# kwea123/nsff_pl

Hardware: AMD Instinct MI355X
Metric: ray-samples/sec (coarse+fine, static+dynamic) (higher is better)
Workload: dtype f16x3 (fp32 operands split into 2 halfs, 3 f16 MFMAs per product, fp32 accumulate; same 1e-4 parity as f32); 1 GPU; C2 (BASELINE.json configs[1]): static+dynamic NSFF, 1024 rays/GPU x (64 coarse + 64 importance -> 192 fine pts), train-mode fwd, fw/bw flow warp t+-1, perturb=1 noise_std=1, 8x256 MLPs, N_tau=48, all 47 outputs on device.  `value` is render_rays' throughput with autograd DISABLED (the train-mode FLAGS, inference launches: nothing kept for a backward pass); what a trainer's forward costs is aux.tra; rays_per_gpu=1024, N_samples=64, N_importance=64, parallelism=single GPU, field_launch=persistent (one workgroup per CU)

## Files before the change

### include/nsff_render.h

```cpp
#ifndef NSFF_RENDER_H
#define NSFF_RENDER_H

#include <stddef.h>
#include <stdint.h>

#ifdef __cplusplus
extern "C" {
#endif

#define NSFF_OK               0
#define NSFF_ERR_INVALID     -1
#define NSFF_ERR_NULL        -2
#define NSFF_ERR_ALIGN       -3
#define NSFF_ERR_HIP         -4

#define NSFF_ABI_VERSION      32
#define NSFF_RAW_STRIDE      16
#define NSFF_MAX_FREQS       24
#define NSFF_MAX_LAYERS       8


typedef struct NsffModelDesc {
    int32_t D;
    int32_t W;
    int32_t skip;
    int32_t in_xyz;
    int32_t in_dir;
    int32_t in_a;
    int32_t in_t;
    int32_t use_viewdir;
    int32_t has_transient;
    int32_t has_flow;
    float   flow_scale;
    int32_t skip_mask;
} NsffModelDesc;

static inline uint32_t nsff_skip_layers(const NsffModelDesc* d) {
    return d->skip_mask ? (uint32_t)d->skip_mask : (d->skip > 0 ? 1u << d->skip : 0u);
}

#define NSFF_PREC_F32        0
#define NSFF_PREC_F16X3      1

int nsff_packed_bytes(const NsffModelDesc* desc, int precision, size_t* bytes);

int nsff_param_count(const NsffModelDesc* desc);

int nsff_pack_weights(const NsffModelDesc* desc, int precision, const float* const* params,
                      void* packed, void* stream);

#define NSFF_PACK_SKIP_FOLD 1
int nsff_pack_weights_ex(const NsffModelDesc* desc, int precision, const float* const* params,
                         void* packed, int32_t flags, void* stream);
int nsff_fold_heads(const NsffModelDesc* desc, int precision, const float* const* params, void* packed, void* stream);

int nsff_posenc(const float* x, int64_t n_rows, const float* freqs_host, int n_freqs,
                float* out, void* stream);

int nsff_time_rows(const float* table, int64_t n_table, int32_t width, const int64_t* ts, int64_t n, int64_t max_t,
                   float* next, float* prev, void* stream);

int nsff_time_rows_backward(const float* g_cur, const float* g_next, const float* g_prev, const int64_t* ts, int64_t n,
                            int64_t max_t, int64_t n_table, int32_t width, float* d_table, void* stream);

typedef struct NsffFieldArgs {
    int64_t n_points;
    int32_t precision;
    int32_t tile_points;
    int32_t pts_per_ray;
    int32_t static_mode;
    int32_t transient_mode;
    int32_t flow_heads;
    const float* xyz;
    int32_t n_freqs;
    float   freqs[NSFF_MAX_FREQS];
    const float* dir_emb;
    const float* a_emb;
    const float* t_emb;
    const float* x_emb;
    int32_t ld_emb;
    int32_t off_xyz, off_dir, off_a, off_t;
    float*  raw;
    void*   save_acts;
    void*   save_xin;
    void*   save_masks;
    void*   save_side;
    const float* t_bias;
    int32_t t_bias_rows;
    int32_t reserved0;
    const float* s_bias;
    int32_t s_bias_rows;
    int32_t launch_form;
    int64_t save_lo_delta[3];
} NsffFieldArgs;

int nsff_field_query(const NsffModelDesc* desc, const void* packed,
                     const NsffFieldArgs* args, void* stream);

#define NSFF_MAX_TIME_BIAS_JOBS 4
typedef struct NsffTimeBiasJob {
    const NsffModelDesc* desc;
    const float* w[NSFF_MAX_LAYERS];
    const float* b[NSFF_MAX_LAYERS];
    const float* t_rows;
    float* out;
    const float* table;
    const int64_t* ts;
    int64_t n_table, max_t;
    int32_t delta, pad_;
    float* rows_out;
} NsffTimeBiasJob;
int nsff_time_bias_rows(const NsffModelDesc* desc);
int nsff_time_bias(const NsffTimeBiasJob* jobs, int32_t n_jobs, int64_t n_rays, void* stream);

#define NSFF_MAX_RNG_JOBS 12
typedef struct NsffRngJob {
    float*   out;
    int64_t  numel;
    uint64_t offset;
    int32_t  kind;
    uint32_t grid;
} NsffRngJob;
int nsff_rng_draws(const NsffRngJob* jobs, int32_t n_jobs, uint64_t seed, void* stream);
typedef struct NsffRngCoarse {
    const float* rays;
    const float* z_lin;
    float*       zs;
    float*       xyz;
    int32_t      n_samples;
    float        perturb;
    int32_t      job;
    int32_t      pad_;
} NsffRngCoarse;
int nsff_rng_draws_coarse(const NsffRngJob* jobs, int32_t n_jobs, uint64_t seed, const NsffRngCoarse* coarse, void* stream);

int nsff_side_bias(const NsffModelDesc* desc, const void* packed_f16x3, const float* w_dir, const float* dir_rows,
                   const float* a_rows, int64_t n_rays, float* out, void* stream);

int nsff_train_dims(const NsffModelDesc* desc, int32_t* xin_rows, int32_t* t_row0, int32_t* side_rows);
int nsff_bwd_packed_bytes(const NsffModelDesc* desc, size_t* bytes);
int nsff_pack_weights_bwd(const NsffModelDesc* desc, const float* const* params, void* packed, void* stream);
int nsff_pack_weights_bwd_ex(const NsffModelDesc* desc, const float* const* params, void* packed, const void* fwd_packed, void* stream);

typedef struct NsffFieldBwdArgs {
    int64_t n_points;
    int32_t static_mode;
    int32_t transient_mode;
    const float* d_raw;
    const float* raw;
    const float* gmax;
    const void*  masks;
    void*  dpre;
    void*  dhead;
    float* d_xin;
    float* d_side;
    int64_t dpre_lo_delta;
} NsffFieldBwdArgs;
int nsff_field_backward(const NsffModelDesc* desc, const void* packed_bwd, const NsffFieldBwdArgs* args, void* stream);
int nsff_last_bwd_kernel(void);
int nsff_last_bwd_grid(void);
int nsff_field_bwd_phase_program(const NsffModelDesc* desc, int32_t dynamic, int32_t want_xin, int64_t n_tiles, uint32_t* out,
                                 int32_t max_phases, uint32_t* seg_offsets, int32_t max_segs);

#define NSFF_BWD_LAUNCH_C    1
#define NSFF_BWD_LAUNCH_H3B  2
#define NSFF_BWD_LAUNCH_X3   3
int nsff_field_bwd_launch_plan(const NsffModelDesc* desc, const NsffFieldBwdArgs* args, int32_t n_cus, int32_t kernel_override,
                               int32_t persist, int32_t* out, int32_t max_launches);

int nsff_field_input_backward(const float* d_xin, int32_t xin_rows, int32_t t_row0, const float* xyz, int64_t n_rays,
                              int32_t pts_per_ray, const float* freqs_host, int32_t n_freqs, int32_t in_t, float* d_xyz,
                              float* d_t, void* stream);

typedef struct NsffWgradJob {
    const void* a;  const void* b;
    int32_t a_rows, b_rows;
    int64_t out_off;
    int32_t trunk, pad_;
    int64_t a_lo_delta, b_lo_delta;
} NsffWgradJob;
int64_t nsff_weight_grad_scratch(const NsffWgradJob* jobs, int32_t n_jobs, int64_t n_tiles, int32_t n_splits);
int nsff_weight_grad(const NsffWgradJob* jobs, int32_t n_jobs, int64_t n_tiles, int32_t n_splits,
                     float* scratch, float* out, float* bias, const float* gmax, void* stream);

typedef struct NsffGradMapEntry {
    int32_t dst;
    int32_t e_a, e_b;
    int16_t job_a, job_b;
} NsffGradMapEntry;
int nsff_weight_grad_accumulate(const NsffWgradJob* jobs, int32_t n_jobs, int64_t n_tiles, int32_t n_splits, float* scratch,
                                const NsffGradMapEntry* map, int64_t n_map, float* grad_base, const float* gmax, void* stream);

int nsff_weight_grad_accumulate_aux(const NsffWgradJob* jobs, int32_t n_jobs, int64_t n_tiles, int32_t n_splits, float* scratch,
                                    const NsffGradMapEntry* map, int64_t n_map, float* grad_base, float* aux, const float* gmax,
                                    void* stream);

typedef struct NsffFoldGradArgs {
    int32_t n_rows, pad_;
    const float* g; const float* gb;
    const float* w_final; const float* b_final;
    const float* w_head[16];
    float* d_w_head[16]; float* d_b_head[16];
    float* d_w_final; float* d_b_final;
} NsffFoldGradArgs;
int nsff_fold_grads(const NsffFoldGradArgs* args, void* stream);

typedef struct NsffFoldDenseArgs {
    int32_t n_rows, accumulate;
    int32_t ld_head, ld_dhead;
    const float* g; const float* g2; const float* gb; const float* gb2;
    const float* w_head; const float* w_final; const float* b_final;
    float* d_w_head; float* d_b_head; float* d_w_final; float* d_b_final;
} NsffFoldDenseArgs;
int nsff_fold_grads_dense(const NsffFoldDenseArgs* args, void* stream);

int nsff_absmax(const float* x, int64_t n, float* out, void* stream);
int nsff_absmax_raw(const float* d_raw, int64_t n_points, float* out16, void* stream);

int nsff_adam_step(float* param, const float* grad, float* exp_avg, float* exp_avg_sq, int64_t n, float* state,
                   const float* lr, double beta1, double beta2, double eps, double weight_decay, void* stream);

int nsff_adam_step_segments(float* param, const float* grad, float* exp_avg, float* exp_avg_sq, int64_t n, float* state,
                            const float* lr, double beta1, double beta2, double eps, double weight_decay,
                            const int64_t* seg_start, int n_seg, int32_t* seg_used, void* stream);

typedef struct NsffLossArgs {
    int64_t n_rays; int32_t n_samples; int32_t n_keep;
    int32_t n_frames; int32_t max_t;
    double  topk;
    int32_t thickness; int32_t pad_;
    const float* rgb_fine; const float* rgb_coarse;
    const float* depth_fine; const float* depth_coarse;
    const float* t_weights; const float* s_weights;
    const float* xyz_fw; const float* xyz_bw;
    const float* rgb_fw; const float* rgb_bw;
    const float* disocc_fw; const float* disocc_bw;
    const float* disoccs_fw; const float* disoccs_bw;
    const float* xyzs_fw_bw; const float* xyzs_bw_fw;
    const float* xyzs_fine; const float* xyzs_fw; const float* xyzs_bw;
    const float* rgbs; const float* disps;
    const int64_t* ts; const int64_t* cam_ids;
    const float* uv_fw; const float* uv_bw;
    const float* Ks; const float* Ps;
    const float* hyper;
    float* stats;
    float* terms;
    const float* term_w;
    const float* weights;
    float* per_ray;
    float* coef;
    float* g_rgb_fine; float* g_rgb_coarse; float* g_depth_fine; float* g_depth_coarse;
    float* g_t_weights; float* g_s_weights; float* g_xyz_fw; float* g_xyz_bw; float* g_rgb_fw; float* g_rgb_bw;
    float* g_xyzs_fw_bw; float* g_xyzs_bw_fw; float* g_xyzs_fw; float* g_xyzs_bw;
} NsffLossArgs;
int nsff_nerfw_loss(const NsffLossArgs* args, int mode, void* stream);
#define NSFF_LOSS_MAX_RAYS 1048576
size_t nsff_nerfw_loss_work_bytes(long long n_rays);
int nsff_nerfw_loss_ex(const NsffLossArgs* args, int mode, void* work, size_t work_bytes, void* stream);
int nsff_last_loss_path(void);

int nsff_coarse_samples(const float* rays, int64_t n_rays, const float* z_lin, int32_t n_samples,
                        float perturb, const float* perturb_rand,
                        float* zs, float* xyz, void* stream);

int nsff_fine_samples(const float* rays, int64_t n_rays, const float* z_lin, const float* zs_coarse,
                      int32_t n_samples, int32_t n_importance,
                      const float* weights_static, const float* weights_transient,
                      const float* u_static, const float* u_transient, int32_t u_per_ray,
                      float* samples_static, float* samples_transient,
                      float* zs_fine, float* xyz_fine, void* stream);

int nsff_sample_pdf(const float* bins, const float* weights, int64_t n_rays, int32_t n_bins_minus1,
                    const float* u, int32_t n_importance, int32_t u_per_ray, float eps,
                    float* samples, void* stream);

int nsff_warp_points(const float* raw, const float* xyz, const float* zs, int64_t n_points,
                     float z_far, float* xyz_fw, float* xyz_bw, void* stream);

int nsff_frame_rays(const float* K4_host, const float* c2w_host, int32_t H, int32_t W, float near, float shift_near,
                    int64_t first_pixel, int64_t n_pixels, float* rays, void* stream);

typedef struct NsffFrustumArgs {
    const float*   w2c;
    const int64_t* ts;
    float   K4[4];
    int32_t n_cams, n_frames, H, W;
} NsffFrustumArgs;

typedef struct NsffCompositeArgs {
    int64_t n_rays;
    int32_t n_samples;
    int32_t has_transient;
    int32_t has_rgb;
    int32_t flow_mode;
    int32_t want_disocc;
    float   noise_std;
    float   z_far;
    const float* raw;
    const float* raw_fw;
    const float* raw_bw;
    const float* zs;
    const float* xyz;
    const float* xyz_fw;
    const float* xyz_bw;
    const float* noise_static;
    const float* noise_transient;
    const float* noise_fw;
    const float* noise_bw;
    const float* visibility;
    float* static_rgbs;  float* transient_rgbs;
    float* flows_fw;     float* flows_bw;
    float* static_sigmas; float* transient_sigmas;
    float* static_alphas; float* transient_alphas;
    float* static_weights; float* transient_weights; float* weights;
    float* xyzs_fw_bw;   float* xyzs_bw_fw;
    float* disoccs_fw;   float* disoccs_bw;
    float* depth;  float* rgb;  float* transient_alpha;  float* transient_rgb;
    float* static_only_rgb;  float* static_only_depth;
    float* xyz_exp;  float* flow_fw_exp;  float* flow_bw_exp;  float* xyz_fw_exp;  float* xyz_bw_exp;
    float* rgb_fw;   float* rgb_bw;
    float* disocc_fw;  float* disocc_bw;
    NsffFrustumArgs vis;
} NsffCompositeArgs;

int nsff_composite(const NsffCompositeArgs* args, void* stream);

int nsff_frustum_visibility(const NsffFrustumArgs* vis, const float* xyz, int64_t n_points, float* vis_count,
                            void* stream);

typedef struct NsffSplatArgs {
    int32_t H, W, n_planes;
    float   K4[4];
    float   P[12];
    float   scale;
    const float* xyz;
    const float* flow;
    const float* rgb;
    const float* alpha;
    float*       accum;
    void*        work;
    int64_t      work_bytes;
} NsffSplatArgs;
int64_t nsff_splat_work_bytes(int32_t H, int32_t W, int32_t n_planes);
int nsff_splat_planes(const NsffSplatArgs* args, void* stream);

typedef struct NsffMpiArgs {
    int32_t H, W, n_planes;
    float   dt;
    const float* accum_fw;
    const float* accum_bw;
    const float* static_rgb;
    const float* static_alpha;
    const float* zs;
    float* rgb;
    float* depth;
} NsffMpiArgs;
int nsff_mpi_composite(const NsffMpiArgs* args, void* stream);

typedef struct NsffCompositeBwdArgs {
    int64_t n_rays;
    int32_t n_samples, has_transient, flow_mode;
    float   noise_std;
    const float* raw;  const float* raw_fw;  const float* raw_bw;
    const float* zs;   const float* xyz;     const float* f_fw;  const float* f_bw;
    const float* noise_static;  const float* noise_transient;  const float* noise_fw;  const float* noise_bw;
    const float* g_static_sigmas;  const float* g_transient_sigmas;
    const float* g_static_weights; const float* g_transient_weights;  const float* g_weights;
    const float* g_depth;  const float* g_rgb;  const float* g_transient_alpha;  const float* g_transient_rgb;
    const float* g_so_rgb; const float* g_so_depth;
    const float* g_xyz_exp;  const float* g_flow_fw_exp;  const float* g_flow_bw_exp;
    const float* g_rgb_fw;   const float* g_rgb_bw;
    float* scratch;
    float* d_raw;  float* d_raw_fw;  float* d_raw_bw;  float* d_f_fw;  float* d_f_bw;
} NsffCompositeBwdArgs;
int nsff_composite_backward(const NsffCompositeBwdArgs* args, void* stream);

typedef struct {
    int64_t n_points;
    const float* zs;
    float z_far;
    int32_t accumulate;
    int32_t col_a, col_b;
    int32_t pad_;
    const float* g_a[4];
    const float* g_b[4];
    float* out;
} NsffFlowGradArgs;
int nsff_flow_grad(const NsffFlowGradArgs* args, void* stream);

#define NSFF_RAY_RECORD      16

typedef struct NsffSsimArgs {
    int32_t n_frames, H, W, window;
    const float* gt;  const float* pred;  const uint8_t* mask;
    float* map;  float* mean_map;  double* sums;
    void* scratch;  int64_t scratch_bytes;
} NsffSsimArgs;
int64_t nsff_ssim_scratch_bytes(int32_t n_frames, int32_t H, int32_t W);
int nsff_ssim(const NsffSsimArgs* args, void* stream);

int nsff_cdf(const float* weights, int64_t n_frames, int64_t n, double* cdf, void* stream);

typedef struct NsffRayDrawArgs {
    int64_t n_frames, n_pixels, frame, batch;
    const float* records;  const double* cdf;  const float* u;
    float* rays;  float* rgbs;  int64_t* ts;  int64_t* cam_ids;  float* disps;  float* rays_mask;  float* uv_fw;  float* uv_bw;
    int64_t* rand_idx;
} NsffRayDrawArgs;
int nsff_ray_draw(const NsffRayDrawArgs* args, void* stream);

int nsff_prof_enable(int on);
int nsff_prof_collect(int64_t* launches, double* total_ms, double* total_flops, double* executed_flops);
int nsff_prof_collect_clock(int64_t* launches, double* total_ms, double* total_flops, double* executed_flops,
                            double* shader_ticks, double* ticks_ms);

#define NSFF_KERNEL_F32       1
#define NSFF_KERNEL_H3_64     2
#define NSFF_KERNEL_H3_8WAVE  3
#define NSFF_KERNEL_H3A       4
#define NSFF_KERNEL_H3_SAVE   5
#define NSFF_KERNEL_H3A_TBIAS 7
#define NSFF_KERNEL_H3A_SAVE  9
#define NSFF_KERNEL_H3A_SIDE  8
int         nsff_last_field_kernel(void);
int         nsff_last_field_grid(void);
int         nsff_field_phase_program(const NsffModelDesc* desc, int static_mode, int transient_mode, int fold_t, uint32_t* steps,
                             int* n_steps, int* n_static_steps, uint32_t* phases_static, uint32_t* phases_dynamic, int* n_phases);

#define NSFF_PLAN_WORDS 12
#define NSFF_LAUNCH_SIDE_TILE      1
#define NSFF_LAUNCH_H3_64          2
#define NSFF_LAUNCH_H3_64_SAVE     3
#define NSFF_LAUNCH_H3_8WAVE       4
#define NSFF_LAUNCH_H3_8WAVE_SAVE  5
#define NSFF_LAUNCH_H3A            6
#define NSFF_LAUNCH_H3A_SAVE       7
int         nsff_field_launch_plan(const NsffModelDesc* desc, const NsffFieldArgs* args, int32_t n_cus, int32_t no_persist,
                                   int32_t* out, int32_t max_launches);

#define NSFF_RANGE_ACT     0x1u
#define NSFF_RANGE_SAVED   0x2u
#define NSFF_RANGE_PARAMS  0x4u
#define NSFF_RANGE_CODES   0x8u
int         nsff_range_flags(uint32_t* out, int32_t clear, void* stream);

int         nsff_abi_version(void);
const char* nsff_last_hip_error(void);

#ifdef __cplusplus
}
#endif
#endif
```

### nsff_pl_amd/_lib.py

```python
import ctypes as C
import os

import torch

_HERE = os.path.dirname(os.path.abspath(__file__))
LIB_PATH = os.environ.get("NSFF_LIB") or os.path.join(_HERE, "libnsff_hip.so")

RAW_STRIDE = 16
ABI_VERSION = 32
MAX_FREQS = 24

_ERR = {-1: "NSFF_ERR_INVALID (bad shape/flag/unsupported architecture)",
        -2: "NSFF_ERR_NULL (required pointer missing)",
        -3: "NSFF_ERR_ALIGN (pointer not 16-byte aligned)",
        -4: "NSFF_ERR_HIP"}

_fp = C.c_void_p


class ModelDesc(C.Structure):
    _fields_ = [("D", C.c_int32), ("W", C.c_int32), ("skip", C.c_int32),
                ("in_xyz", C.c_int32), ("in_dir", C.c_int32), ("in_a", C.c_int32),
                ("in_t", C.c_int32), ("use_viewdir", C.c_int32),
                ("has_transient", C.c_int32), ("has_flow", C.c_int32),
                ("flow_scale", C.c_float), ("skip_mask", C.c_int32)]


class FieldArgs(C.Structure):
    _fields_ = [("n_points", C.c_int64), ("precision", C.c_int32), ("tile_points", C.c_int32),
                ("pts_per_ray", C.c_int32),
                ("static_mode", C.c_int32), ("transient_mode", C.c_int32),
                ("flow_heads", C.c_int32),
                ("xyz", _fp), ("n_freqs", C.c_int32), ("freqs", C.c_float * MAX_FREQS),
                ("dir_emb", _fp), ("a_emb", _fp), ("t_emb", _fp),
                ("x_emb", _fp), ("ld_emb", C.c_int32),
                ("off_xyz", C.c_int32), ("off_dir", C.c_int32), ("off_a", C.c_int32),
                ("off_t", C.c_int32), ("raw", _fp), ("save_acts", _fp), ("save_xin", _fp), ("save_masks", _fp),
                ("save_side", _fp), ("t_bias", _fp), ("t_bias_rows", C.c_int32), ("reserved0", C.c_int32),
                ("s_bias", _fp), ("s_bias_rows", C.c_int32), ("launch_form", C.c_int32), ("save_lo_delta", C.c_int64 * 3)]


class TimeBiasJob(C.Structure):
    _fields_ = [("desc", C.POINTER(ModelDesc)), ("w", _fp * 8), ("b", _fp * 8), ("t_rows", _fp), ("out", _fp),
                ("table", _fp), ("ts", _fp), ("n_table", C.c_int64), ("max_t", C.c_int64), ("delta", C.c_int32), ("pad_", C.c_int32),
                ("rows_out", _fp)]


MAX_TIME_BIAS_JOBS = 4


class RngJob(C.Structure):
    _fields_ = [("out", _fp), ("numel", C.c_int64), ("offset", C.c_uint64), ("kind", C.c_int32), ("grid", C.c_uint32)]


MAX_RNG_JOBS = 12


class RngCoarse(C.Structure):
    _fields_ = [("rays", _fp), ("z_lin", _fp), ("zs", _fp), ("xyz", _fp), ("n_samples", C.c_int32), ("perturb", C.c_float),
                ("job", C.c_int32), ("pad_", C.c_int32)]


_COMPOSITE_PTRS_IN = ["raw", "raw_fw", "raw_bw", "zs", "xyz", "xyz_fw", "xyz_bw",
                      "noise_static", "noise_transient", "noise_fw", "noise_bw", "visibility"]
_COMPOSITE_PTRS_OUT = ["static_rgbs", "transient_rgbs", "flows_fw", "flows_bw",
                       "static_sigmas", "transient_sigmas", "static_alphas", "transient_alphas",
                       "static_weights", "transient_weights", "weights",
                       "xyzs_fw_bw", "xyzs_bw_fw", "disoccs_fw", "disoccs_bw",
                       "depth", "rgb", "transient_alpha", "transient_rgb",
                       "static_only_rgb", "static_only_depth",
                       "xyz_exp", "flow_fw_exp", "flow_bw_exp", "xyz_fw_exp", "xyz_bw_exp",
                       "rgb_fw", "rgb_bw", "disocc_fw", "disocc_bw"]


class FrustumArgs(C.Structure):
    _fields_ = [("w2c", _fp), ("ts", _fp), ("K4", C.c_float * 4), ("n_cams", C.c_int32), ("n_frames", C.c_int32),
                ("H", C.c_int32), ("W", C.c_int32)]


class CompositeArgs(C.Structure):
    _fields_ = ([("n_rays", C.c_int64), ("n_samples", C.c_int32), ("has_transient", C.c_int32),
                 ("has_rgb", C.c_int32), ("flow_mode", C.c_int32), ("want_disocc", C.c_int32),
                 ("noise_std", C.c_float), ("z_far", C.c_float)]
                + [(n, _fp) for n in _COMPOSITE_PTRS_IN]
                + [(n, _fp) for n in _COMPOSITE_PTRS_OUT]
                + [("vis", FrustumArgs)])


_CBWD_IN = ["raw", "raw_fw", "raw_bw", "zs", "xyz", "f_fw", "f_bw", "noise_static", "noise_transient", "noise_fw", "noise_bw"]
_CBWD_G = ["g_static_sigmas", "g_transient_sigmas", "g_static_weights", "g_transient_weights", "g_weights", "g_depth",
           "g_rgb", "g_transient_alpha", "g_transient_rgb", "g_so_rgb", "g_so_depth", "g_xyz_exp", "g_flow_fw_exp",
           "g_flow_bw_exp", "g_rgb_fw", "g_rgb_bw"]
_CBWD_OUT = ["scratch", "d_raw", "d_raw_fw", "d_raw_bw", "d_f_fw", "d_f_bw"]


class CompositeBwdArgs(C.Structure):
    _fields_ = ([("n_rays", C.c_int64), ("n_samples", C.c_int32), ("has_transient", C.c_int32), ("flow_mode", C.c_int32),
                 ("noise_std", C.c_float)] + [(n, _fp) for n in _CBWD_IN + _CBWD_G + _CBWD_OUT])


class FieldBwdArgs(C.Structure):
    _fields_ = [("n_points", C.c_int64), ("static_mode", C.c_int32), ("transient_mode", C.c_int32),
                ("d_raw", _fp), ("raw", _fp), ("gmax", _fp), ("masks", _fp), ("dpre", _fp), ("dhead", _fp),
                ("d_xin", _fp), ("d_side", _fp), ("dpre_lo_delta", C.c_int64)]


class WgradJob(C.Structure):
    _fields_ = [("a", _fp), ("b", _fp), ("a_rows", C.c_int32), ("b_rows", C.c_int32), ("out_off", C.c_int64), ("trunk", C.c_int32),
                ("pad_", C.c_int32), ("a_lo_delta", C.c_int64), ("b_lo_delta", C.c_int64)]


class FoldGradArgs(C.Structure):
    _fields_ = [("n_rows", C.c_int32), ("pad_", C.c_int32), ("g", _fp), ("gb", _fp), ("w_final", _fp), ("b_final", _fp),
                ("w_head", _fp * 16), ("d_w_head", _fp * 16), ("d_b_head", _fp * 16), ("d_w_final", _fp), ("d_b_final", _fp)]


class FoldDenseArgs(C.Structure):
    _fields_ = [("n_rows", C.c_int32), ("accumulate", C.c_int32), ("ld_head", C.c_int32), ("ld_dhead", C.c_int32),
                ("g", _fp), ("g2", _fp), ("gb", _fp), ("gb2", _fp), ("w_head", _fp), ("w_final", _fp), ("b_final", _fp),
                ("d_w_head", _fp), ("d_b_head", _fp), ("d_w_final", _fp), ("d_b_final", _fp)]


class SplatArgs(C.Structure):
    _fields_ = [("H", C.c_int32), ("W", C.c_int32), ("n_planes", C.c_int32), ("K4", C.c_float * 4),
                ("P", C.c_float * 12), ("scale", C.c_float),
                ("xyz", _fp), ("flow", _fp), ("rgb", _fp), ("alpha", _fp), ("accum", _fp), ("work", _fp),
                ("work_bytes", C.c_int64)]


class MpiArgs(C.Structure):
    _fields_ = [("H", C.c_int32), ("W", C.c_int32), ("n_planes", C.c_int32), ("dt", C.c_float),
                ("accum_fw", _fp), ("accum_bw", _fp), ("static_rgb", _fp), ("static_alpha", _fp), ("zs", _fp),
                ("rgb", _fp), ("depth", _fp)]


_LOSS_IN = ["rgb_fine", "rgb_coarse", "depth_fine", "depth_coarse", "t_weights", "s_weights", "xyz_fw", "xyz_bw", "rgb_fw",
            "rgb_bw", "disocc_fw", "disocc_bw", "disoccs_fw", "disoccs_bw", "xyzs_fw_bw", "xyzs_bw_fw", "xyzs_fine",
            "xyzs_fw", "xyzs_bw", "rgbs", "disps", "ts", "cam_ids", "uv_fw", "uv_bw", "Ks", "Ps", "hyper", "stats", "terms",
            "term_w"]
LOSS_GRADS = ["g_rgb_fine", "g_rgb_coarse", "g_depth_fine", "g_depth_coarse", "g_t_weights", "g_s_weights", "g_xyz_fw",
              "g_xyz_bw", "g_rgb_fw", "g_rgb_bw", "g_xyzs_fw_bw", "g_xyzs_bw_fw", "g_xyzs_fw", "g_xyzs_bw"]


class LossArgs(C.Structure):
    _fields_ = ([("n_rays", C.c_int64), ("n_samples", C.c_int32), ("n_keep", C.c_int32), ("n_frames", C.c_int32),
                 ("max_t", C.c_int32), ("topk", C.c_double), ("thickness", C.c_int32), ("pad_", C.c_int32)]
                + [(n, _fp) for n in _LOSS_IN] + [("weights", _fp), ("per_ray", _fp), ("coef", _fp)]
                + [(n, _fp) for n in LOSS_GRADS])


class FlowGradArgs(C.Structure):
    _fields_ = [("n_points", C.c_int64), ("zs", _fp), ("z_far", C.c_float), ("accumulate", C.c_int32), ("col_a", C.c_int32),
                ("col_b", C.c_int32), ("pad_", C.c_int32), ("g_a", _fp * 4), ("g_b", _fp * 4), ("out", _fp)]


class SsimArgs(C.Structure):
    _fields_ = [("n_frames", C.c_int32), ("H", C.c_int32), ("W", C.c_int32), ("window", C.c_int32),
                ("gt", _fp), ("pred", _fp), ("mask", _fp), ("map", _fp), ("mean_map", _fp), ("sums", _fp),
                ("scratch", _fp), ("scratch_bytes", C.c_int64)]


RAY_RECORD = 16
_DRAW_OUT = ["rays", "rgbs", "ts", "cam_ids", "disps", "rays_mask", "uv_fw", "uv_bw", "rand_idx"]


class RayDrawArgs(C.Structure):
    _fields_ = ([("n_frames", C.c_int64), ("n_pixels", C.c_int64), ("frame", C.c_int64), ("batch", C.c_int64),
                 ("records", _fp), ("cdf", _fp), ("u", _fp)] + [(n, _fp) for n in _DRAW_OUT])


_SIGNATURES = {
    "nsff_abi_version": (C.c_int, []),
    "nsff_range_flags": (C.c_int, [_fp, C.c_int32, _fp]),
    "nsff_last_field_kernel": (C.c_int, []),
    "nsff_last_field_grid": (C.c_int, []),
    "nsff_field_phase_program": (C.c_int, [C.POINTER(ModelDesc), C.c_int, C.c_int, C.c_int, C.POINTER(C.c_uint32), C.POINTER(C.c_int),
                                   C.POINTER(C.c_int), C.POINTER(C.c_uint32), C.POINTER(C.c_uint32), C.POINTER(C.c_int)]),
    "nsff_field_launch_plan": (C.c_int, [C.POINTER(ModelDesc), C.POINTER(FieldArgs), C.c_int32, C.c_int32, C.POINTER(C.c_int32), C.c_int32]),
    "nsff_time_bias_rows": (C.c_int, [C.POINTER(ModelDesc)]),
    "nsff_time_bias": (C.c_int, [C.POINTER(TimeBiasJob), C.c_int32, C.c_int64, C.c_void_p]),
    "nsff_rng_draws": (C.c_int, [C.POINTER(RngJob), C.c_int32, C.c_uint64, C.c_void_p]),
    "nsff_rng_draws_coarse": (C.c_int, [C.POINTER(RngJob), C.c_int32, C.c_uint64, C.POINTER(RngCoarse), C.c_void_p]),
    "nsff_side_bias": (C.c_int, [C.POINTER(ModelDesc), _fp, _fp, _fp, _fp, C.c_int64, _fp, C.c_void_p]),
    "nsff_last_hip_error": (C.c_char_p, []),
    "nsff_packed_bytes": (C.c_int, [C.POINTER(ModelDesc), C.c_int, C.POINTER(C.c_size_t)]),
    "nsff_param_count": (C.c_int, [C.POINTER(ModelDesc)]),
    "nsff_pack_weights": (C.c_int, [C.POINTER(ModelDesc), C.c_int, C.POINTER(_fp), _fp, _fp]),
    "nsff_pack_weights_ex": (C.c_int, [C.POINTER(ModelDesc), C.c_int, C.POINTER(_fp), _fp, C.c_int32, _fp]),
    "nsff_fold_heads": (C.c_int, [C.POINTER(ModelDesc), C.c_int, C.POINTER(_fp), _fp, _fp]),
    "nsff_posenc": (C.c_int, [_fp, C.c_int64, C.POINTER(C.c_float), C.c_int, _fp, _fp]),
    "nsff_time_rows": (C.c_int, [_fp, C.c_int64, C.c_int32, _fp, C.c_int64, C.c_int64, _fp, _fp, _fp]),
    "nsff_time_rows_backward": (C.c_int, [_fp, _fp, _fp, _fp, C.c_int64, C.c_int64, C.c_int64, C.c_int32, _fp, _fp]),
    "nsff_field_query": (C.c_int, [C.POINTER(ModelDesc), _fp, C.POINTER(FieldArgs), _fp]),
    "nsff_coarse_samples": (C.c_int, [_fp, C.c_int64, _fp, C.c_int32, C.c_float, _fp, _fp, _fp, _fp]),
    "nsff_fine_samples": (C.c_int, [_fp, C.c_int64, _fp, _fp, C.c_int32, C.c_int32, _fp, _fp, _fp, _fp,
                                    C.c_int32, _fp, _fp, _fp, _fp, _fp]),
    "nsff_sample_pdf": (C.c_int, [_fp, _fp, C.c_int64, C.c_int32, _fp, C.c_int32, C.c_int32,
                                  C.c_float, _fp, _fp]),
    "nsff_warp_points": (C.c_int, [_fp, _fp, _fp, C.c_int64, C.c_float, _fp, _fp, _fp]),
    "nsff_composite": (C.c_int, [C.POINTER(CompositeArgs), _fp]),
    "nsff_frustum_visibility": (C.c_int, [C.POINTER(FrustumArgs), _fp, C.c_int64, _fp, _fp]),
    "nsff_frame_rays": (C.c_int, [C.POINTER(C.c_float), C.POINTER(C.c_float), C.c_int32, C.c_int32, C.c_float,
                                  C.c_float, C.c_int64, C.c_int64, _fp, _fp]),
    "nsff_bwd_packed_bytes": (C.c_int, [C.POINTER(ModelDesc), C.POINTER(C.c_size_t)]),
    "nsff_pack_weights_bwd": (C.c_int, [C.POINTER(ModelDesc), C.POINTER(_fp), _fp, _fp]),
    "nsff_field_backward": (C.c_int, [C.POINTER(ModelDesc), _fp, C.POINTER(FieldBwdArgs), _fp]),
    "nsff_field_input_backward": (C.c_int, [_fp, C.c_int32, C.c_int32, _fp, C.c_int64, C.c_int32, C.POINTER(C.c_float), C.c_int32,
                                            C.c_int32, _fp, _fp, _fp]),
    "nsff_train_dims": (C.c_int, [C.POINTER(ModelDesc), C.POINTER(C.c_int32), C.POINTER(C.c_int32), C.POINTER(C.c_int32)]),
    "nsff_weight_grad_scratch": (C.c_int64, [C.POINTER(WgradJob), C.c_int32, C.c_int64, C.c_int32]),
    "nsff_weight_grad": (C.c_int, [C.POINTER(WgradJob), C.c_int32, C.c_int64, C.c_int32, _fp, _fp, _fp, _fp, _fp]),
    "nsff_weight_grad_accumulate": (C.c_int, [C.POINTER(WgradJob), C.c_int32, C.c_int64, C.c_int32, _fp, _fp, C.c_int64,
                                              _fp, _fp, _fp]),
    "nsff_weight_grad_accumulate_aux": (C.c_int, [C.POINTER(WgradJob), C.c_int32, C.c_int64, C.c_int32, _fp, _fp, C.c_int64,
                                                  _fp, _fp, _fp, _fp]),
    "nsff_absmax_raw": (C.c_int, [_fp, C.c_int64, _fp, _fp]),
    "nsff_last_bwd_kernel": (C.c_int, []),
    "nsff_last_bwd_grid": (C.c_int, []),
    "nsff_field_bwd_phase_program": (C.c_int, [C.POINTER(ModelDesc), C.c_int32, C.c_int32, C.c_int64, C.POINTER(C.c_uint32), C.c_int32,
                                                C.POINTER(C.c_uint32), C.c_int32]),
    "nsff_field_bwd_launch_plan": (C.c_int, [C.POINTER(ModelDesc), C.POINTER(FieldBwdArgs), C.c_int32, C.c_int32, C.c_int32,
                                             C.POINTER(C.c_int32), C.c_int32]),
    "nsff_fold_grads": (C.c_int, [C.POINTER(FoldGradArgs), _fp]),
    "nsff_fold_grads_dense": (C.c_int, [C.POINTER(FoldDenseArgs), _fp]),
    "nsff_pack_weights_bwd_ex": (C.c_int, [C.POINTER(ModelDesc), C.POINTER(_fp), _fp, _fp, _fp]),
    "nsff_absmax": (C.c_int, [_fp, C.c_int64, _fp, _fp]),
    "nsff_adam_step": (C.c_int, [_fp, _fp, _fp, _fp, C.c_int64, _fp, _fp, C.c_double, C.c_double, C.c_double, C.c_double, _fp]),
    "nsff_adam_step_segments": (C.c_int, [_fp, _fp, _fp, _fp, C.c_int64, _fp, _fp, C.c_double, C.c_double, C.c_double, C.c_double,
                                          _fp, C.c_int, _fp, _fp]),
    "nsff_composite_backward": (C.c_int, [C.POINTER(CompositeBwdArgs), _fp]),
    "nsff_flow_grad": (C.c_int, [C.POINTER(FlowGradArgs), _fp]),
    "nsff_nerfw_loss": (C.c_int, [C.POINTER(LossArgs), C.c_int, _fp]),
    "nsff_nerfw_loss_work_bytes": (C.c_size_t, [C.c_longlong]),
    "nsff_nerfw_loss_ex": (C.c_int, [C.POINTER(LossArgs), C.c_int, _fp, C.c_size_t, _fp]),
    "nsff_last_loss_path": (C.c_int, []),
    "nsff_splat_planes": (C.c_int, [C.POINTER(SplatArgs), _fp]),
    "nsff_splat_work_bytes": (C.c_int64, [C.c_int32, C.c_int32, C.c_int32]),
    "nsff_mpi_composite": (C.c_int, [C.POINTER(MpiArgs), _fp]),
    "nsff_ssim_scratch_bytes": (C.c_int64, [C.c_int32, C.c_int32, C.c_int32]),
    "nsff_ssim": (C.c_int, [C.POINTER(SsimArgs), _fp]),
    "nsff_cdf": (C.c_int, [_fp, C.c_int64, C.c_int64, _fp, _fp]),
    "nsff_ray_draw": (C.c_int, [C.POINTER(RayDrawArgs), _fp]),
    "nsff_prof_enable": (C.c_int, [C.c_int]),
    "nsff_prof_collect": (C.c_int, [C.POINTER(C.c_int64), C.POINTER(C.c_double), C.POINTER(C.c_double), C.POINTER(C.c_double)]),
    "nsff_prof_collect_clock": (C.c_int, [C.POINTER(C.c_int64)] + [C.POINTER(C.c_double)] * 5),
}
EXPORTED_SYMBOLS = tuple(_SIGNATURES)

_lib = None


def load():
    global _lib
    if _lib is None:
        if not os.path.exists(LIB_PATH):
            raise RuntimeError(
                f"{LIB_PATH} is missing: build it with `python -c 'import __graft_entry__ as g; g.build()'` "
                "(or `make -C nsff_pl_amd/csrc`).  There is no CPU fallback for the render path.")
        lib = C.CDLL(LIB_PATH)
        for name, (res, args) in _SIGNATURES.items():
            fn = getattr(lib, name)
            fn.restype, fn.argtypes = res, args
        if lib.nsff_abi_version() != ABI_VERSION:
            raise RuntimeError("libnsff_hip.so ABI version mismatch")
        _lib = lib
    return _lib


def _check(rc, what):
    if rc != 0:
        msg = _ERR.get(rc, f"error {rc}")
        if rc == -4:
            msg += ": " + load().nsff_last_hip_error().decode()
        raise RuntimeError(f"{what} failed: {msg}")


def require_gpu_tensor(t, what):
    if not isinstance(t, torch.Tensor) or not t.is_cuda:
        raise RuntimeError(f"{what} must be a GPU tensor: the NSFF render path runs only on the "
                           "HIP kernels of libnsff_hip.so (no CPU fallback)")


def _ptr(t):
    if t is None:
        return None
    assert t.is_cuda and t.dtype == torch.float32 and t.is_contiguous(), "need contiguous fp32 GPU tensor"
    return t.data_ptr()


def _stream():
    return torch.cuda.current_stream().cuda_stream


def model_desc(model):
    if model.W != 256:
        raise RuntimeError(f"unsupported NeRF architecture: W={model.W} (the gfx950 field kernels tile W=256 trunks "
                           "into 4 x 64-neuron wave blocks; other widths are not built)")
    skips = sorted(set(int(s) for s in model.skips))
    if not 2 <= model.D <= 8 or any(not 1 <= s < model.D for s in skips):
        raise RuntimeError(f"unsupported NeRF architecture: D={model.D}, skips={list(model.skips)} (need 2 <= D <= 8 "
                           "and every skip layer in 1..D-1; a skip at layer 0 would concatenate the input with itself)")
    mask = sum(1 << s for s in skips)
    return ModelDesc(D=model.D, W=model.W, skip=skips[0] if len(skips) == 1 else 0, skip_mask=mask if len(skips) != 1 else 0,
                     in_xyz=model.in_channels_xyz,
                     in_dir=model.in_channels_dir,
                     in_a=model.in_channels_a if model.use_viewdir else 0,
                     in_t=model.in_channels_t, use_viewdir=int(model.use_viewdir),
                     has_transient=int(model.encode_transient),
                     has_flow=int(getattr(model, "has_flow_heads", hasattr(model, "transient_flow_fw"))),
                     flow_scale=float(getattr(model, "flow_scale", 0.0)))


def param_list(model):
    def lin(m):
        layer = m[0] if isinstance(m, torch.nn.Sequential) else m
        return [layer.weight, layer.bias]
    out = []
    for i in range(model.D):
        out += lin(getattr(model, f"static_xyz_encoding_{i + 1}"))
    out += lin(model.static_xyz_encoding_final)
    if model.use_viewdir:
        out += lin(model.static_dir_encoding)
    out += lin(model.static_sigma) + lin(model.static_rgb)
    if model.encode_transient:
        for i in range(model.D):
            out += lin(getattr(model, f"transient_xyz_encoding_{i + 1}"))
        out += lin(model.transient_xyz_encoding_final)
        out += lin(model.transient_sigma) + lin(model.transient_rgb)
        if hasattr(model, "transient_flow_fw"):
            out += lin(model.transient_flow_fw) + lin(model.transient_flow_bw)
    return out


def packed_bytes(desc, precision=0):
    n = C.c_size_t(0)
    _check(load().nsff_packed_bytes(C.byref(desc), int(precision), C.byref(n)), "nsff_packed_bytes")
    return n.value


PACK_SKIP_FOLD = 1


def pack_weights(desc, params, packed, precision=0, fold=True):
    lib = load()
    if lib.nsff_param_count(C.byref(desc)) != len(params):
        raise RuntimeError("parameter list does not match the model description")
    keep = [p.detach().contiguous().float() for p in params]
    for p in keep:
        require_gpu_tensor(p, "model parameter")
    arr = (_fp * len(keep))(*[p.data_ptr() for p in keep])
    _check(lib.nsff_pack_weights_ex(C.byref(desc), int(precision), arr, _ptr(packed), 0 if fold else PACK_SKIP_FOLD,
                                    _stream()), "nsff_pack_weights_ex")
    return keep


def fold_heads(desc, params, packed, precision):
    keep = [p.detach().contiguous().float() for p in params]
    arr = (_fp * len(keep))(*[p.data_ptr() for p in keep])
    _check(load().nsff_fold_heads(C.byref(desc), int(precision), arr, _ptr(packed), _stream()), "nsff_fold_heads")
    return keep


def time_rows_backward(g_cur, g_next, g_prev, ts, max_t, n_table):
    gs = [None if g is None else g.contiguous() for g in (g_cur, g_next, g_prev)]
    width = next(g for g in gs if g is not None).shape[1]
    assert ts.dtype == torch.int64 and ts.is_cuda and ts.is_contiguous()
    d = torch.empty(int(n_table), width, device=ts.device)
    _check(load().nsff_time_rows_backward(_ptr(gs[0]), _ptr(gs[1]), _ptr(gs[2]), C.c_void_p(ts.data_ptr()), ts.shape[0],
                                          int(max_t), int(n_table), width, _ptr(d), _stream()), "nsff_time_rows_backward")
    return d


def time_rows(table, ts, max_t, want_next=True, want_prev=True):
    n, width = ts.shape[0], table.shape[1]
    if want_next and want_prev:
        both = torch.empty(2, n, width, device=table.device)
        nxt, prv = both[0], both[1]
    else:
        nxt = torch.empty(n, width, device=table.device) if want_next else None
        prv = torch.empty(n, width, device=table.device) if want_prev else None
    assert ts.dtype == torch.int64 and ts.is_cuda and ts.is_contiguous()
    _check(load().nsff_time_rows(_ptr(table), table.shape[0], width, C.c_void_p(ts.data_ptr()), n, int(max_t),
                                 _ptr(nxt), _ptr(prv), _stream()), "nsff_time_rows")
    return nxt, prv


def posenc(x, freqs, out):
    f = [float(v) for v in freqs]
    arr = (C.c_float * len(f))(*f)
    _check(load().nsff_posenc(_ptr(x), x.shape[0], arr, len(f), _ptr(out), _stream()), "nsff_posenc")


def field_query(model, raw, n_points, pts_per_ray, static_mode, transient_mode, flow_heads=0,
                xyz=None, freqs=None, dir_emb=None, a_emb=None, t_emb=None,
                x_emb=None, emb_offsets=(0, -1, -1, -1), save_acts=None, save_xin=None, save_masks=None, save_side=None,
                precision=None, t_bias=None, s_bias=None, save_lo=False):
    from . import config
    desc = model_desc(model)
    prec = config.precision_code(model) if precision is None else precision
    saves = not (save_acts is None and save_xin is None and save_masks is None and save_side is None)
    packed = model.packed(prec)
    a = FieldArgs()
    a.precision, a.tile_points = prec, config.get_tile_points()
    a.launch_form = 0 if config.get_persistent() else 1
    a.n_points, a.pts_per_ray = int(n_points), int(pts_per_ray)
    a.static_mode, a.transient_mode, a.flow_heads = int(static_mode), int(transient_mode), int(flow_heads)
    a.xyz = _ptr(xyz)
    if freqs is not None:
        f = [float(v) for v in freqs]
        if len(f) > MAX_FREQS:
            raise RuntimeError("too many embedding frequencies")
        a.n_freqs = len(f)
        for i, v in enumerate(f):
            a.freqs[i] = v
    a.dir_emb, a.a_emb, a.t_emb = _ptr(dir_emb), _ptr(a_emb), _ptr(t_emb)
    a.x_emb = _ptr(x_emb)
    a.ld_emb = int(x_emb.shape[1]) if x_emb is not None else 0
    a.off_xyz, a.off_dir, a.off_a, a.off_t = [int(v) for v in emb_offsets]
    a.raw = _ptr(raw)
    a.save_acts = None if save_acts is None else save_acts.data_ptr()
    a.save_xin = None if save_xin is None else save_xin.data_ptr()
    a.save_masks = None if save_masks is None else save_masks.data_ptr()
    a.save_side = None if save_side is None else save_side.data_ptr()
    if save_lo:
        for i, t in enumerate((save_acts, save_xin, save_side)):
            a.save_lo_delta[i] = 0 if t is None else lo_delta(t)
    if t_bias is not None:
        a.t_bias, a.t_bias_rows = _ptr(t_bias), int(t_bias.shape[1])
    if s_bias is not None:
        a.s_bias, a.s_bias_rows = _ptr(s_bias), int(s_bias.shape[1])
    _check(load().nsff_field_query(C.byref(desc), _ptr(packed), C.byref(a), _stream()), "nsff_field_query")


def lo_delta(t):
    n = t.numel()
    if t.untyped_storage().nbytes() < (t.storage_offset() + 2 * n) * t.element_size():
        raise RuntimeError("three-product backward: this buffer has no remainder plane behind it (field_grad.alloc_saves(..., x3=True))")
    return n


def side_bias(model, dir_rows, a_rows=None):
    from . import config
    desc = model_desc(model)
    n_rays = int(dir_rows.shape[0])
    assert dir_rows.shape == (n_rays, desc.in_dir) and (desc.in_a == 0 or (a_rows is not None and a_rows.shape == (n_rays, desc.in_a)))
    packed = model.packed(config.PRECISIONS["f16x3"])
    w = model.static_dir_encoding[0].weight.detach()
    out = torch.empty(n_rays, 1, 256, device=dir_rows.device, dtype=torch.float32)
    _check(load().nsff_side_bias(C.byref(desc), _ptr(packed), _ptr(w), _ptr(dir_rows), _ptr(a_rows) if desc.in_a > 0 else None,
                                 n_rays, _ptr(out), _stream()), "nsff_side_bias")
    return out


_DEVICE_RNG_GEOMETRY = {}


def fused_draws(plan, device, values=True, coarse=None):
    dev = torch.device(device)
    idx = dev.index if dev.index is not None else torch.cuda.current_device()
    if idx not in _DEVICE_RNG_GEOMETRY:
        p = torch.cuda.get_device_properties(idx)
        _DEVICE_RNG_GEOMETRY[idx] = p.multi_processor_count * (p.max_threads_per_multi_processor // 256)
    max_grid = _DEVICE_RNG_GEOMETRY[idx]
    gen = torch.cuda.default_generators[idx]
    seed, offset = gen.initial_seed(), gen.get_offset()
    wanted = values if isinstance(values, (list, tuple)) else [bool(values)] * len(plan)
    sizes = []
    for kind, shape in plan:
        n = 1
        for s in shape:
            n *= int(s)
        sizes.append(n)
    total = sum(n for n, w in zip(sizes, wanted) if w)
    buf = torch.empty(max(total, 1), device=dev, dtype=torch.float32)
    outs, jobs, at = [], [], 0
    for (kind, shape), numel, want in zip(plan, sizes, wanted):
        if numel == 0:
            outs.append(torch.empty(*shape, device=dev, dtype=torch.float32))
            continue
        grid = min(max_grid, (numel + 255) // 256)
        if coarse is not None and not outs and not want:
            jobs.append((None, numel, offset, 0, grid))
            outs.append(None)
        elif want:
            t = buf[at:at + numel].view(*shape)
            at += numel
            jobs.append((t, numel, offset, 1 if kind == "randn" else 0, grid))
            outs.append(t)
        else:
            outs.append(None)
        offset += ((numel - 1) // (1024 * grid) + 1) * 4
    hook = None
    if coarse is not None:
        rays, z_lin, perturb, zs, xyz = coarse
        assert plan and plan[0][0] == "rand" and tuple(plan[0][1]) == (rays.shape[0], z_lin.shape[0]) and perturb > 0
        if sizes[0]:
            hook = RngCoarse(_ptr(rays), _ptr(z_lin), _ptr(zs), _ptr(xyz), int(z_lin.shape[0]), float(perturb), 0, 0)
    for k in range(0, len(jobs), MAX_RNG_JOBS):
        part = jobs[k:k + MAX_RNG_JOBS]
        arr = (RngJob * len(part))()
        for j, (t, numel, off, kind, grid) in enumerate(part):
            arr[j].out, arr[j].numel, arr[j].offset, arr[j].kind, arr[j].grid = (None if t is None else t.data_ptr()), numel, off, kind, grid
        with torch.cuda.device(idx):
            _check(load().nsff_rng_draws_coarse(arr, len(part), seed, C.byref(hook) if (hook is not None and k == 0) else None, _stream()),
                   "nsff_rng_draws")
    gen.set_offset(offset)
    return outs


_FUSED_DRAWS_OK = {}


def fused_draws_match_torch(device):
    dev = torch.device(device)
    idx = dev.index if dev.index is not None else torch.cuda.current_device()
    if idx in _FUSED_DRAWS_OK:
        return _FUSED_DRAWS_OK[idx]
    if torch.cuda.is_current_stream_capturing():
        return False
    gen = torch.cuda.default_generators[idx]
    state = gen.get_state()
    ok = True
    try:
        plan = [("rand", (7, 64)), ("randn", (1031,)), ("rand", (3, 5, 2)), ("randn", (70000,)), ("rand", (300001,))]
        gen.manual_seed(0x5EED1234)
        gen.set_offset(8)
        mine = fused_draws(plan, torch.device("cuda", idx))
        end_mine = gen.get_offset()
        gen.manual_seed(0x5EED1234)
        gen.set_offset(8)
        with torch.cuda.device(idx):
            ref = [(torch.rand if k == "rand" else torch.randn)(*shape, device=torch.device("cuda", idx)) for k, shape in plan]
        end_ref = gen.get_offset()
        ok = end_mine == end_ref and all(torch.equal(a.view(torch.int32), b.view(torch.int32)) for a, b in zip(mine, ref))
    except Exception:
        ok = False
    finally:
        gen.set_state(state)
    if not ok:
        import warnings
        warnings.warn("nsff_pl_amd: the fused generator kernel (nsff_rng_draws) no longer reproduces torch.rand / torch.randn on "
                      f"cuda:{idx} (torch {torch.__version__}); render_rays draws with the torch calls instead (slower by ~1 %, same "
                      "numbers as the reference)")
    _FUSED_DRAWS_OK[idx] = ok
    return ok


def time_bias_rows(model):
    return load().nsff_time_bias_rows(C.byref(model_desc(model)))


def time_bias(jobs, index=None):
    assert 1 <= len(jobs) <= MAX_TIME_BIAS_JOBS
    arr = (TimeBiasJob * len(jobs))()
    keep, outs, per_model, pair = [], [], {}, None
    rows_of = {}
    if index is not None:
        table, ts, max_t = index
        assert ts.dtype == torch.int64 and ts.is_cuda and ts.is_contiguous() and ts.dim() == 1, "ts: one int64 frame index per ray"
        n_rays, width = int(ts.shape[0]), int(table.shape[1])
        deltas = sorted({int(d) for _, d in jobs})
        if 1 in deltas and -1 in deltas:
            both = torch.empty(2, n_rays, width, device=table.device, dtype=torch.float32)
            rows_of[1], rows_of[-1] = both[0], both[1]
        for d in deltas:
            if d not in rows_of:
                rows_of[d] = torch.empty(n_rays, width, device=table.device, dtype=torch.float32)
        written = set()
    else:
        n_rays = int(jobs[0][1].shape[0])
    for j, (model, t_rows) in enumerate(jobs):
        if id(model) not in per_model:
            desc = model_desc(model)
            lins = [getattr(model, f"transient_xyz_encoding_{l + 1}")[0] for l in [0] + sorted(set(int(v) for v in model.skips))]
            wb = [(m.weight.detach(), m.bias.detach()) for m in lins]
            for w, b in wb:
                _ptr(w), _ptr(b)
            per_model[id(model)] = (desc, C.pointer(desc), wb)
        desc, pdesc, wb = per_model[id(model)]
        if index is not None:
            delta, t_rows = int(t_rows), None
            assert width == desc.in_t
        else:
            assert t_rows.shape == (n_rays, desc.in_t)
        dev = wb[0][0].device
        if j + 1 < len(jobs) and jobs[j + 1][0] is model and pair is None:
            pair = torch.empty(2, n_rays, len(wb), 256, device=dev, dtype=torch.float32)
            out = pair[0]
        elif pair is not None:
            out, pair = pair[1], None
        else:
            out = torch.empty(n_rays, len(wb), 256, device=dev, dtype=torch.float32)
        arr[j].desc = pdesc
        for i, (w, b) in enumerate(wb):
            arr[j].w[i], arr[j].b[i] = w.data_ptr(), b.data_ptr()
        arr[j].t_rows, arr[j].out = _ptr(t_rows), _ptr(out)
        if index is not None:
            arr[j].table, arr[j].ts = _ptr(table), ts.data_ptr()
            arr[j].n_table, arr[j].max_t, arr[j].delta = int(table.shape[0]), int(max_t), delta
            if delta not in written:
                arr[j].rows_out = _ptr(rows_of[delta])
                written.add(delta)
        outs.append(out)
    keep.append(per_model)
    _check(load().nsff_time_bias(arr, len(jobs), n_rays, _stream()), "nsff_time_bias")
    return outs if index is None else (outs, rows_of)


def coarse_samples(rays, z_lin, perturb, perturb_rand, zs, xyz):
    _check(load().nsff_coarse_samples(_ptr(rays), rays.shape[0], _ptr(z_lin), z_lin.shape[0],
                                      float(perturb), _ptr(perturb_rand), _ptr(zs), _ptr(xyz), _stream()),
           "nsff_coarse_samples")


def fine_samples(rays, z_lin, zs_coarse, n_importance, w_static, w_transient, u_static, u_transient,
                 u_per_ray, samples_static, samples_transient, zs_fine, xyz_fine):
    _check(load().nsff_fine_samples(_ptr(rays), rays.shape[0], _ptr(z_lin), _ptr(zs_coarse),
                                    z_lin.shape[0], int(n_importance), _ptr(w_static), _ptr(w_transient),
                                    _ptr(u_static), _ptr(u_transient), int(u_per_ray),
                                    _ptr(samples_static), _ptr(samples_transient),
                                    _ptr(zs_fine), _ptr(xyz_fine), _stream()), "nsff_fine_samples")


def sample_pdf(bins, weights, u, u_per_ray, eps, samples):
    _check(load().nsff_sample_pdf(_ptr(bins), _ptr(weights), weights.shape[0], weights.shape[1],
                                  _ptr(u), samples.shape[1], int(u_per_ray), float(eps),
                                  _ptr(samples), _stream()), "nsff_sample_pdf")


def warp_points(raw, xyz, zs, z_far, xyz_fw, xyz_bw):
    _check(load().nsff_warp_points(_ptr(raw), _ptr(xyz), _ptr(zs), zs.numel(), float(z_far),
                                   _ptr(xyz_fw), _ptr(xyz_bw), _stream()), "nsff_warp_points")


def frustum_args(w2c, ts, K4, n_cams, n_frames, H, W):
    assert w2c.is_cuda and w2c.dtype == torch.float32 and w2c.is_contiguous() and w2c.shape == (n_cams * n_frames, 12)
    assert ts.is_cuda and ts.dtype == torch.int64 and ts.is_contiguous() and ts.numel() >= 1
    a = FrustumArgs(w2c=w2c.data_ptr(), ts=ts.data_ptr(), n_cams=int(n_cams), n_frames=int(n_frames), H=int(H), W=int(W))
    a.K4[:] = [float(v) for v in K4]
    a._keep = (w2c, ts)
    return a


def frustum_visibility(vis, xyz, out):
    _check(load().nsff_frustum_visibility(C.byref(vis), _ptr(xyz), xyz.shape[0], _ptr(out), _stream()),
           "nsff_frustum_visibility")


def composite(vis=None, **kw):
    a = CompositeArgs()
    for k, v in kw.items():
        if k in _COMPOSITE_PTRS_IN or k in _COMPOSITE_PTRS_OUT:
            setattr(a, k, _ptr(v))
        else:
            setattr(a, k, v)
    if vis is not None:
        a.vis = vis
    _check(load().nsff_composite(C.byref(a), _stream()), "nsff_composite")


def frame_rays(K4, c2w12, H, W, near, shift_near, first, count, rays):
    k = (C.c_float * 4)(*[float(v) for v in K4])
    m = (C.c_float * 12)(*[float(v) for v in c2w12])
    _check(load().nsff_frame_rays(k, m, int(H), int(W), float(near), float(shift_near), int(first), int(count),
                                  _ptr(rays), _stream()), "nsff_frame_rays")


BWD_PACK = 100


def bwd_packed_bytes(desc):
    n = C.c_size_t(0)
    _check(load().nsff_bwd_packed_bytes(C.byref(desc), C.byref(n)), "nsff_bwd_packed_bytes")
    return n.value


def pack_weights_bwd(desc, params, packed, fwd_packed=None):
    arr = (_fp * len(params))(*[p.data_ptr() for p in params])
    _check(load().nsff_pack_weights_bwd_ex(C.byref(desc), arr, _ptr(packed), _ptr(fwd_packed), _stream()), "nsff_pack_weights_bwd_ex")


def last_bwd_kernel():
    return {0: "c", 1: "h3b", 2: "c+h3b", 3: "x3"}[load().nsff_last_bwd_kernel()]


def last_bwd_grid():
    return load().nsff_last_bwd_grid()


PLAN_WORDS = 12


def field_launch_plan(desc, args, n_cus, no_persist=False):
    out = (C.c_int32 * (3 * PLAN_WORDS))()
    code = load().nsff_field_launch_plan(C.byref(desc), C.byref(args), int(n_cus), int(bool(no_persist)), out, 3)
    recs = [list(out[i * PLAN_WORDS:(i + 1) * PLAN_WORDS]) for i in range(3)]
    return code, [r for r in recs if r[0] != 0]


def field_bwd_launch_plan(desc, args, n_cus, kernel_override=None, persist=True):
    out = (C.c_int32 * (2 * PLAN_WORDS))()
    code = load().nsff_field_bwd_launch_plan(C.byref(desc), C.byref(args), int(n_cus), ord(kernel_override) if kernel_override else 0,
                                                      int(bool(persist)), out, 2)
    recs = [list(out[i * PLAN_WORDS:(i + 1) * PLAN_WORDS]) for i in range(2)]
    return code, [r for r in recs if r[0] != 0]


def field_bwd_phase_program(model, dynamic, want_xin, n_tiles, max_phases=32):
    import numpy as np
    desc = model_desc(model)
    out = (C.c_uint32 * (8 * max_phases))()
    segs = (C.c_uint32 * 48)()
    n = load().nsff_field_bwd_phase_program(C.byref(desc), 1 if dynamic else 0, 1 if want_xin else 0, int(n_tiles), out, max_phases, segs, 48)
    if n < 0:
        raise RuntimeError(f"nsff_field_bwd_phase_program failed ({n})")
    offs = np.array(list(segs), np.uint32)
    return (np.array(list(out), np.uint32).reshape(max_phases, 8)[:n] if n > 0 else None), offs


def field_backward(model, n_points, static, transient, d_raw, raw, gmax, masks, dpre, dhead, d_xin, d_side=None, x3=False):
    desc = model_desc(model)
    a = FieldBwdArgs(n_points=int(n_points), static_mode=2 if static else 0, transient_mode=2 if transient else 0,
                     d_raw=_ptr(d_raw), raw=_ptr(raw), gmax=_ptr(gmax), masks=masks.data_ptr(), dpre=dpre.data_ptr(),
                     dhead=dhead.data_ptr(), d_xin=_ptr(d_xin), d_side=_ptr(d_side), dpre_lo_delta=lo_delta(dpre) if x3 else 0)
    _check(load().nsff_field_backward(C.byref(desc), _ptr(model.packed(BWD_PACK)), C.byref(a), _stream()),
           "nsff_field_backward")


def train_dims(model):
    desc = model_desc(model)
    xr, t0, sr = C.c_int32(0), C.c_int32(0), C.c_int32(0)
    _check(load().nsff_train_dims(C.byref(desc), C.byref(xr), C.byref(t0), C.byref(sr)), "nsff_train_dims")
    return xr.value, t0.value, sr.value


def field_input_backward(d_xin, t_row0, xyz, pts_per_ray, freqs, in_t, want_xyz, want_t):
    P, xin_rows = d_xin.shape
    n_rays = P // pts_per_ray
    d_xyz = torch.empty(P, 3, device=d_xin.device) if want_xyz else None
    d_t = torch.empty(n_rays, in_t, device=d_xin.device) if want_t else None
    f = [float(v) for v in freqs]
    arr = (C.c_float * max(len(f), 1))(*f)
    _check(load().nsff_field_input_backward(_ptr(d_xin), int(xin_rows), int(t_row0), _ptr(xyz), n_rays, int(pts_per_ray), arr,
                                            len(f), int(in_t), _ptr(d_xyz), _ptr(d_t), _stream()), "nsff_field_input_backward")
    return d_xyz, d_t


def _wgrad_jobs(jobs, with_off):
    return (WgradJob * len(jobs))(*[WgradJob(a=j[0], b=j[1], a_rows=j[2], b_rows=j[3], out_off=j[4] if with_off else 0, trunk=j[5],
                                             a_lo_delta=j[6] if len(j) > 6 else 0, b_lo_delta=j[7] if len(j) > 7 else 0) for j in jobs])


def weight_grad(jobs, n_tiles, n_splits, out, bias, gmax):
    arr = _wgrad_jobs(jobs, True)
    n = load().nsff_weight_grad_scratch(arr, len(jobs), int(n_tiles), int(n_splits))
    if n < 0:
        raise RuntimeError("nsff_weight_grad_scratch failed")
    scratch = torch.empty(n, device=out.device)
    _check(load().nsff_weight_grad(arr, len(jobs), int(n_tiles), int(n_splits), _ptr(scratch), _ptr(out), _ptr(bias),
                                   _ptr(gmax), _stream()), "nsff_weight_grad")


def weight_grad_accumulate(jobs, n_tiles, n_splits, grad_map, grad_base_ptr, gmax, aux=None):
    arr = _wgrad_jobs(jobs, False)
    n = load().nsff_weight_grad_scratch(arr, len(jobs), int(n_tiles), int(n_splits))
    if n < 0:
        raise RuntimeError("nsff_weight_grad_scratch failed")
    assert grad_map.dtype == torch.int32 and grad_map.is_contiguous() and grad_map.shape[1] == 4
    scratch = torch.empty(n, device=gmax.device)
    _check(load().nsff_weight_grad_accumulate_aux(arr, len(jobs), int(n_tiles), int(n_splits), _ptr(scratch),
                                                  C.c_void_p(grad_map.data_ptr()), grad_map.shape[0], C.c_void_p(grad_base_ptr),
                                                  _ptr(aux), _ptr(gmax), _stream()), "nsff_weight_grad_accumulate_aux")
    return scratch


def fold_grads(g, gb, w_final, b_final, head_rows, d_w_final, d_b_final):
    a = FoldGradArgs(n_rows=len(head_rows), g=_ptr(g), gb=_ptr(gb), w_final=_ptr(w_final), b_final=_ptr(b_final),
                     d_w_final=_ptr(d_w_final), d_b_final=_ptr(d_b_final))
    for r, (w, dw, db) in enumerate(head_rows):
        a.w_head[r], a.d_w_head[r], a.d_b_head[r] = w.data_ptr(), dw.data_ptr(), db.data_ptr()
    _check(load().nsff_fold_grads(C.byref(a), _stream()), "nsff_fold_grads")


def fold_grads_dense(g, gb, w_head, w_final, b_final, d_w_head, d_b_head, d_w_final, d_b_final, accumulate, g2=None, gb2=None):
    R = int(g.shape[0])
    for t in (g, g2, gb, gb2, w_final, b_final, d_w_final, d_b_final, d_b_head):
        assert t is None or (t.is_cuda and t.dtype == torch.float32 and t.is_contiguous())
    for t in (w_head, d_w_head):
        assert t.is_cuda and t.dtype == torch.float32 and t.shape[0] == R and t.shape[1] == 256 and t.stride(1) == 1
    a = FoldDenseArgs(n_rows=R, accumulate=1 if accumulate else 0, ld_head=int(w_head.stride(0)), ld_dhead=int(d_w_head.stride(0)),
                      g=g.data_ptr(), g2=None if g2 is None else g2.data_ptr(), gb=gb.data_ptr(), gb2=None if gb2 is None else gb2.data_ptr(),
                      w_head=w_head.data_ptr(), w_final=w_final.data_ptr(), b_final=b_final.data_ptr(), d_w_head=d_w_head.data_ptr(),
                      d_b_head=d_b_head.data_ptr(), d_w_final=d_w_final.data_ptr(), d_b_final=d_b_final.data_ptr())
    _check(load().nsff_fold_grads_dense(C.byref(a), _stream()), "nsff_fold_grads_dense")


def absmax(x):
    x = x.contiguous()
    if x.dim() == 2 and x.shape[1] == RAW_STRIDE:
        out = torch.empty(RAW_STRIDE, device=x.device, dtype=torch.float32)
        _check(load().nsff_absmax_raw(_ptr(x), x.shape[0], _ptr(out), _stream()), "nsff_absmax_raw")
        return out
    out = torch.empty((), device=x.device, dtype=torch.float32)
    _check(load().nsff_absmax(_ptr(x), x.numel(), _ptr(out), _stream()), "nsff_absmax")
    return out


def adam_step(param, grad, exp_avg, exp_avg_sq, state, lr, beta1, beta2, eps, weight_decay, seg_start=None, seg_used=None):
    if seg_start is None:
        _check(load().nsff_adam_step(_ptr(param), _ptr(grad), _ptr(exp_avg), _ptr(exp_avg_sq), param.numel(), _ptr(state), _ptr(lr),
                                     float(beta1), float(beta2), float(eps), float(weight_decay), _stream()), "nsff_adam_step")
        return
    _check(load().nsff_adam_step_segments(_ptr(param), _ptr(grad), _ptr(exp_avg), _ptr(exp_avg_sq), param.numel(), _ptr(state),
                                          _ptr(lr), float(beta1), float(beta2), float(eps), float(weight_decay),
                                          C.c_void_p(seg_start.data_ptr()), int(seg_used.numel()),
                                          C.c_void_p(seg_used.data_ptr()), _stream()),
           "nsff_adam_step_segments")


def composite_backward(n_rays, n_samples, has_transient, flow_mode, noise_std, **tensors):
    a = CompositeBwdArgs(n_rays=int(n_rays), n_samples=int(n_samples), has_transient=int(has_transient),
                         flow_mode=int(flow_mode), noise_std=float(noise_std))
    for k, v in tensors.items():
        setattr(a, k, _ptr(v))
    _check(load().nsff_composite_backward(C.byref(a), _stream()), "nsff_composite_backward")


def flow_grad(zs, z_far, out, accumulate, col_a=-1, g_a=(), col_b=-1, g_b=()):
    a = FlowGradArgs(n_points=int(out.shape[0]), zs=_ptr(zs), z_far=float(z_far), accumulate=int(bool(accumulate)),
                     col_a=int(col_a), col_b=int(col_b), out=_ptr(out))
    if len(g_a) > 4 or len(g_b) > 4:
        raise ValueError("flow_grad: at most four cotangents per group")
    keep = [g.contiguous() for g in list(g_a) + list(g_b)]
    for i, g in enumerate(keep[:len(g_a)]):
        a.g_a[i] = _ptr(g)
    for i, g in enumerate(keep[len(g_a):]):
        a.g_b[i] = _ptr(g)
    _check(load().nsff_flow_grad(C.byref(a), _stream()), "nsff_flow_grad")


def nerfw_loss(mode, n_rays, n_samples, n_keep, n_frames, max_t, topk=1.0, thickness=1, work=None, **tensors):
    a = LossArgs(n_rays=int(n_rays), n_samples=int(n_samples), n_keep=int(n_keep), n_frames=int(n_frames), max_t=int(max_t),
                 topk=float(topk), thickness=int(thickness))
    for k, v in tensors.items():
        if v is None:
            continue
        if not torch.is_tensor(v):
            raise TypeError(f"nerfw_loss: {k} must be a tensor")
        if v.dtype == torch.int64:
            assert v.is_cuda and v.is_contiguous()
            setattr(a, k, v.data_ptr())
        else:
            setattr(a, k, _ptr(v))
    if work is None:
        _check(load().nsff_nerfw_loss(C.byref(a), int(mode), _stream()), "nsff_nerfw_loss")
        return
    if not (torch.is_tensor(work) and work.is_cuda and work.dtype == torch.uint8 and work.is_contiguous()):
        raise TypeError("nerfw_loss: work must be a contiguous uint8 GPU tensor")
    _check(load().nsff_nerfw_loss_ex(C.byref(a), int(mode), work.data_ptr(), work.numel(), _stream()), "nsff_nerfw_loss_ex")


LOSS_MAX_RAYS = 1 << 20


def nerfw_loss_work_bytes(n_rays):
    return int(load().nsff_nerfw_loss_work_bytes(int(n_rays)))


def last_loss_path():
    return int(load().nsff_last_loss_path())


def splat_work_bytes(H, W, S):
    return int(load().nsff_splat_work_bytes(int(H), int(W), int(S)))


def splat_planes(H, W, S, K4, P12, scale, xyz, flow, rgb, alpha, accum, work=None):
    a = SplatArgs(H=int(H), W=int(W), n_planes=int(S), scale=float(scale), xyz=_ptr(xyz), flow=_ptr(flow),
                  rgb=_ptr(rgb), alpha=_ptr(alpha), accum=_ptr(accum))
    if work is not None:
        assert work.is_cuda and work.is_contiguous() and work.dtype == torch.uint8
        a.work, a.work_bytes = work.data_ptr(), work.numel()
    a.K4[:] = [float(v) for v in K4]
    a.P[:] = [float(v) for v in P12]
    _check(load().nsff_splat_planes(C.byref(a), _stream()), "nsff_splat_planes")


def mpi_composite(H, W, S, dt, accum_fw, accum_bw, static_rgb, static_alpha, zs, rgb, depth):
    a = MpiArgs(H=int(H), W=int(W), n_planes=int(S), dt=float(dt), accum_fw=_ptr(accum_fw), accum_bw=_ptr(accum_bw),
                static_rgb=_ptr(static_rgb), static_alpha=_ptr(static_alpha), zs=_ptr(zs), rgb=_ptr(rgb),
                depth=_ptr(depth))
    _check(load().nsff_mpi_composite(C.byref(a), _stream()), "nsff_mpi_composite")


KERNEL_NAMES = {0: None, 1: "f32", 2: "h3_64", 3: "h3_8wave", 4: "h3a", 5: "h3_save", 7: "h3a_tb", 8: "h3a_side", 9: "h3a_save"}


def _dptr(t, dtype, what):
    if t is None:
        return None
    require_gpu_tensor(t, what)
    if t.dtype != dtype or not t.is_contiguous():
        raise RuntimeError(f"{what}: need a contiguous {dtype} tensor, got {t.dtype}"
                           f"{'' if t.is_contiguous() else ' (non-contiguous)'}")
    return t.data_ptr()


def ssim_scratch_bytes(n_frames, H, W):
    return int(load().nsff_ssim_scratch_bytes(int(n_frames), int(H), int(W)))


def ssim(gt, pred, mask=None, map=None, mean_map=None, sums=None, scratch=None):
    require_gpu_tensor(gt, "ssim: image_gt")
    require_gpu_tensor(pred, "ssim: image_pred")
    if gt.dim() != 4 or gt.shape[-1] != 3 or pred.shape != gt.shape:
        raise RuntimeError(f"ssim: need (F, H, W, 3) image pairs of one shape, got {tuple(gt.shape)} and {tuple(pred.shape)}")
    F, H, W = (int(v) for v in gt.shape[:3])
    if mask is not None and mask.dtype == torch.bool:
        mask = mask.view(torch.uint8)
    if sums is not None and scratch is None:
        scratch = torch.zeros(max(ssim_scratch_bytes(F, H, W), 16), dtype=torch.uint8, device=gt.device)
    a = SsimArgs(n_frames=F, H=H, W=W, window=11, gt=_dptr(gt, torch.float32, "ssim: image_gt"),
                 pred=_dptr(pred, torch.float32, "ssim: image_pred"), mask=_dptr(mask, torch.uint8, "ssim: mask"),
                 map=_dptr(map, torch.float32, "ssim: map"), mean_map=_dptr(mean_map, torch.float32, "ssim: mean_map"),
                 sums=_dptr(sums, torch.float64, "ssim: sums"), scratch=_dptr(scratch, torch.uint8, "ssim: scratch"),
                 scratch_bytes=0 if scratch is None else scratch.numel())
    for t, n in ((mask, F * H * W), (map, F * H * W * 3), (mean_map, F * H * W), (sums, F * 3)):
        if t is not None and t.numel() != n:
            raise RuntimeError(f"ssim: an output / mask has {t.numel()} elements, expected {n}")
    with torch.cuda.device(gt.device):
        _check(load().nsff_ssim(C.byref(a), _stream()), "nsff_ssim")


def cdf(weights, out):
    F, N = weights.shape
    if tuple(out.shape) != (F, N):
        raise RuntimeError("cdf: output shape mismatch")
    with torch.cuda.device(weights.device):
        _check(load().nsff_cdf(_dptr(weights, torch.float32, "cdf: weights"), F, N, _dptr(out, torch.float64, "cdf: out"),
                               _stream()), "nsff_cdf")


def ray_draw(records, frame, u, cdf, out):
    NF, NP = int(records.shape[0]), int(records.shape[1])
    if records.dim() != 3 or records.shape[2] != RAY_RECORD:
        raise RuntimeError(f"ray_draw: records must be (N_frames, N_pixels, {RAY_RECORD})")
    B = int(u.numel())
    a = RayDrawArgs(n_frames=NF, n_pixels=NP, frame=int(frame), batch=B, records=_dptr(records, torch.float32, "ray_draw: records"),
                    cdf=_dptr(cdf, torch.float64, "ray_draw: cdf"), u=_dptr(u, torch.float32, "ray_draw: u"))
    for n in _DRAW_OUT:
        t = out.get(n)
        setattr(a, n, _dptr(t, torch.int64 if n in ("ts", "cam_ids", "rand_idx") else torch.float32, f"ray_draw: {n}"))
    with torch.cuda.device(records.device):
        _check(load().nsff_ray_draw(C.byref(a), _stream()), "nsff_ray_draw")


def range_flags(out, clear):
    assert out.is_cuda and out.dtype == torch.int32 and out.numel() >= 1
    _check(load().nsff_range_flags(out.data_ptr(), 1 if clear else 0, _stream()), "nsff_range_flags")


def last_field_kernel():
    return KERNEL_NAMES[load().nsff_last_field_kernel()]


def last_field_grid():
    return int(load().nsff_last_field_grid())


def h3a_program(model, static_mode, transient_mode, fold_t=False, side_fold=False, persist=False):
    desc = model_desc(model)
    steps = (C.c_uint32 * (28 * 4))()
    ps, pd = (C.c_uint32 * (36 * 8))(), (C.c_uint32 * (36 * 8))()
    n, ns, nph = C.c_int(0), C.c_int(0), (C.c_int * 2)()
    _check(load().nsff_field_phase_program(C.byref(desc), int(static_mode), int(transient_mode), int(bool(fold_t)) | (2 if side_fold else 0) | (4 if persist else 0), steps, C.byref(n), C.byref(ns), ps, pd, nph),
           "nsff_field_phase_program")
    out = []
    for i in range(n.value):
        w, b, packed = steps[4 * i], steps[4 * i + 1], steps[4 * i + 2]
        out.append((w, None if b == 0xFFFFFFFF else b, packed & 0xFF, (packed >> 8) & 0xFF, (packed >> 16) & 0xFF, packed >> 24))
    rows = lambda arr, k: [[int(arr[8 * i + j]) for j in range(8)] for i in range(k)]
    return out, ns.value, rows(ps, nph[0]), rows(pd, nph[1])


def prof_enable(on):
    _check(load().nsff_prof_enable(int(bool(on))), "nsff_prof_enable")


def prof_collect():
    n, ms, fl, ex, tk, tms = C.c_int64(0), C.c_double(0), C.c_double(0), C.c_double(0), C.c_double(0), C.c_double(0)
    _check(load().nsff_prof_collect_clock(C.byref(n), C.byref(ms), C.byref(fl), C.byref(ex), C.byref(tk), C.byref(tms)),
           "nsff_prof_collect_clock")
    ghz = tk.value / tms.value * 1e-6 if tms.value > 0 else None
    if ghz is not None and not (0.5 < ghz < 3.0):
        ghz = None
    return n.value, ms.value, fl.value, ex.value, ghz
```

### nsff_pl_amd/csrc/rays.hip

```cpp
#include <hip/hip_runtime.h>
#include <cstdlib>
#include "nsff_common.h"

namespace {

constexpr int WAVES_PER_BLOCK = 4;
constexpr int RS = NSFF_RAW_STRIDE;

__device__ __forceinline__ float wave_sum(float v) {
#pragma unroll
    for (int off = 32; off > 0; off >>= 1) v += __shfl_xor(v, off);
    return v;
}

__device__ __forceinline__ float wave_scan_mul(float v, int lane) {
#pragma unroll
    for (int off = 1; off < 64; off <<= 1) {
        const float u = __shfl_up(v, off);
        if (lane >= off) v *= u;
    }
    return v;
}
__device__ __forceinline__ float wave_scan_add(float v, int lane) {
#pragma unroll
    for (int off = 1; off < 64; off <<= 1) {
        const float u = __shfl_up(v, off);
        if (lane >= off) v += u;
    }
    return v;
}

__device__ __forceinline__ float softplus(float x) { return x > 20.f ? x : log1pf(expf(x)); }

__global__ void coarse_samples_kernel(const float* __restrict__ rays, long long n_rays,
                                      const float* __restrict__ z_lin, int S, float perturb,
                                      const float* __restrict__ rnd, float* __restrict__ zs,
                                      float* __restrict__ xyz) {
    const long long idx = (long long)blockIdx.x * blockDim.x + threadIdx.x;
    if (idx >= n_rays * S) return;
    const long long n = idx / S;
    const int i = (int)(idx - n * S);
    float z = z_lin[i];
    if (perturb > 0.f) {
        const float lower = i > 0 ? 0.5f * (z_lin[i - 1] + z_lin[i]) : z_lin[0];
        const float upper = i < S - 1 ? 0.5f * (z_lin[i] + z_lin[i + 1]) : z_lin[S - 1];
        z = lower + (upper - lower) * (perturb * rnd[idx]);
    }
    zs[idx] = z;
    const float* r = rays + n * 6;
#pragma unroll
    for (int c = 0; c < 3; ++c) xyz[idx * 3 + c] = r[c] + r[3 + c] * z;
}

__device__ __forceinline__ void sample_pdf_ray(const float* w, const float* bins, int M, float eps,
                                               const float* u, int n_imp, float* cdf,
                                               float* out_a, float* out_b, int lane, bool active) {
    float part = 0.f;
    for (int j = lane; j < M; j += 64) part += (active ? w[j] : 0.f) + eps;
    const float total = wave_sum(part);
    float carry = 0.f;
    if (lane == 0) cdf[0] = 0.f;
    for (int base = 0; base < M; base += 64) {
        const int j = base + lane;
        const float pdf = j < M ? ((active ? w[j] : 0.f) + eps) / total : 0.f;
        const float inc = wave_scan_add(pdf, lane) + carry;
        if (j < M) cdf[j + 1] = inc;
        carry = __shfl(inc, 63);
    }
    __syncthreads();
    for (int k = lane; k < n_imp; k += 64) {
        const float uk = active ? u[k] : 0.f;
        int lo = 0, hi = M + 1;
        while (lo < hi) {
            const int mid = (lo + hi) >> 1;
            if (cdf[mid] <= uk) lo = mid + 1; else hi = mid;
        }
        const int below = max(lo - 1, 0), above = min(lo, M);
        const float cb = cdf[below], ca = cdf[above];
        const float bb = bins[below], ba = bins[above];
        float denom = ca - cb;
        if (denom < eps) denom = 1.f;
        const float s = bb + (uk - cb) / denom * (ba - bb);
        if (active) {
            if (out_a) out_a[k] = s;
            if (out_b) out_b[k] = s;
        }
    }
    __syncthreads();
}

struct FineArgs {
    const float* rays; long long n_rays; const float* z_lin; const float* zs_coarse;
    int S, n_imp;
    const float* w_static; const float* w_transient;
    const float* u_static; const float* u_transient; int u_per_ray;
    float* samples_static; float* samples_transient;
    float* zs_fine; float* xyz_fine;
};

__global__ __launch_bounds__(64 * WAVES_PER_BLOCK) void fine_samples_kernel(const FineArgs a) {
    extern __shared__ __attribute__((aligned(16))) float smem[];
    const int lane = threadIdx.x & 63, wave = threadIdx.x >> 6, tid = threadIdx.x;
    constexpr int T = 64 * WAVES_PER_BLOCK;
    const long long ray = blockIdx.x;
    const int S = a.S, n_imp = a.n_imp;
    const int k_sets = a.w_transient ? 2 : 1;
    const int Sf = S + k_sets * n_imp;
    float* cdf = smem + wave * S;
    float* bins = smem + WAVES_PER_BLOCK * S;
    float* merged = bins + ((S + 3) & ~3);
    for (int j = tid; j < S - 1; j += T) bins[j] = 0.5f * (a.z_lin[j] + a.z_lin[j + 1]);
    for (int j = tid; j < S; j += T) merged[j] = a.zs_coarse[ray * S + j];
    __syncthreads();
    {
        const bool mine = wave < k_sets;
        const int set = mine ? wave : 0;
        const float* w = (set == 0 ? a.w_static : a.w_transient) + ray * S + 1;
        const float* ub = set == 0 ? a.u_static : a.u_transient;
        const float* u = a.u_per_ray ? ub + ray * n_imp : ub;
        float* keep = set == 0 ? a.samples_static : a.samples_transient;
        sample_pdf_ray(w, bins, S - 2, 1e-5f, u, n_imp, cdf, merged + S + set * n_imp,
                       keep ? keep + ray * n_imp : nullptr, lane, mine);
    }
    const float* r = a.rays + ray * 6;
    const float o0 = r[0], o1 = r[1], o2 = r[2], d0 = r[3], d1 = r[4], d2 = r[5];
    for (int i = tid; i < Sf; i += T) {
        const float v = merged[i];
        int rank = 0;
        int j = 0;
        for (; j + 4 <= Sf; j += 4) {
            const float4 o = *reinterpret_cast<const float4*>(merged + j);
            rank += (o.x < v || (o.x == v && j < i)) ? 1 : 0;
            rank += (o.y < v || (o.y == v && j + 1 < i)) ? 1 : 0;
            rank += (o.z < v || (o.z == v && j + 2 < i)) ? 1 : 0;
            rank += (o.w < v || (o.w == v && j + 3 < i)) ? 1 : 0;
        }
        for (; j < Sf; ++j) {
            const float o = merged[j];
            rank += (o < v || (o == v && j < i)) ? 1 : 0;
        }
        const long long dst = ray * Sf + rank;
        a.zs_fine[dst] = v;
        a.xyz_fine[dst * 3 + 0] = o0 + d0 * v;
        a.xyz_fine[dst * 3 + 1] = o1 + d1 * v;
        a.xyz_fine[dst * 3 + 2] = o2 + d2 * v;
    }
}

struct PdfArgs {
    const float* bins; const float* weights; long long n_rays; int M;
    const float* u; int n_imp; int u_per_ray; float eps; float* samples;
};

__global__ __launch_bounds__(64 * WAVES_PER_BLOCK) void sample_pdf_kernel(const PdfArgs a) {
    extern __shared__ __attribute__((aligned(16))) float smem[];
    const int lane = threadIdx.x & 63, wave = threadIdx.x >> 6;
    const long long ray_raw = (long long)blockIdx.x * WAVES_PER_BLOCK + wave;
    const bool active = ray_raw < a.n_rays;
    const long long ray = active ? ray_raw : a.n_rays - 1;
    float* cdf = smem + wave * (a.M + 1);
    const float* u = a.u_per_ray ? a.u + ray * a.n_imp : a.u;
    sample_pdf_ray(a.weights + ray * a.M, a.bins + ray * (a.M + 1), a.M, a.eps, u, a.n_imp, cdf,
                   active ? a.samples + ray * a.n_imp : nullptr, nullptr, lane, true);
}

struct FrameRayArgs {
    float fx, fy, cx, cy;
    float c2w[12];
    int W;
    float near, shift_near;
    long long first, count;
    float* rays;
};

__global__ void frame_rays_kernel(const FrameRayArgs a) {
    const long long idx = (long long)blockIdx.x * blockDim.x + threadIdx.x;
    if (idx >= a.count) return;
    const long long pix = a.first + idx;
    const float i = (float)(pix % a.W), j = (float)(pix / a.W);
    const float dc[3] = {(i - a.cx) / a.fx, -(j - a.cy) / a.fy, -1.0f};
    float d[3];
#pragma unroll
    for (int r = 0; r < 3; ++r) d[r] = dc[0] * a.c2w[4 * r + 0] + dc[1] * a.c2w[4 * r + 1] + dc[2] * a.c2w[4 * r + 2];
    const float nrm = sqrtf(d[0] * d[0] + d[1] * d[1] + d[2] * d[2]);
#pragma unroll
    for (int r = 0; r < 3; ++r) d[r] /= nrm;
    float o[3] = {a.c2w[3], a.c2w[7], a.c2w[11]};
    const float t = -(a.shift_near + o[2]) / d[2];
#pragma unroll
    for (int r = 0; r < 3; ++r) o[r] = o[r] + t * d[r];
    const float ox_oz = o[0] / o[2], oy_oz = o[1] / o[2];
    const float sx = -1.0f / (a.cx / a.fx), sy = -1.0f / (a.cy / a.fy);
    const float o2 = 1.0f + 2.0f * a.near / o[2];
    float* r = a.rays + idx * 6;
    r[0] = sx * ox_oz;
    r[1] = sy * oy_oz;
    r[2] = o2;
    r[3] = sx * (d[0] / d[2] - ox_oz);
    r[4] = sy * (d[1] / d[2] - oy_oz);
    r[5] = 1.0f - o2;
}

__global__ void warp_points_kernel(const float* __restrict__ raw, const float* __restrict__ xyz,
                                   const float* __restrict__ zs, long long n_points, float z_far,
                                   float* __restrict__ xyz_fw, float* __restrict__ xyz_bw) {
    const long long idx = (long long)blockIdx.x * blockDim.x + threadIdx.x;
    if (idx >= n_points * 3) return;
    const long long p = idx / 3;
    const int c = (int)(idx - p * 3);
    const bool far = zs[p] > z_far;
    const float x = xyz[idx];
    xyz_fw[idx] = x + (far ? 0.f : raw[p * RS + 8 + c]);
    xyz_bw[idx] = x + (far ? 0.f : raw[p * RS + 11 + c]);
}

__device__ __forceinline__ float frustum_count(const NsffFrustumArgs& v, float x, float y, float z) {
    const float fx = v.K4[0], fy = v.K4[1], cx = v.K4[2], cy = v.K4[3];
    const float rz = 2.0f / (z - 1.0f - 1e-6f);
    const float rx = -rz * x * cx / fx;
    const float ry = -rz * y * cy / fy;
    const long long frame = v.ts[0];
    float count = 0.f;
    if (frame < 0 || frame >= v.n_frames) return count;
    for (int c = 0; c < v.n_cams; ++c) {
        const float* m = v.w2c + ((long long)c * v.n_frames + frame) * 12;
        const float cam0 = fmaf(m[2], rz, fmaf(m[1], ry, m[0] * rx)) + m[3];
        const float cam1 = fmaf(m[6], rz, fmaf(m[5], ry, m[4] * rx)) + m[7];
        const float cam2 = fmaf(m[10], rz, fmaf(m[9], ry, m[8] * rx)) + m[11];
        if (!(cam2 < 0.f)) continue;
        const float c1 = -cam1, c2 = -cam2;
        const float u = fmaf(cx, c2, fx * cam0) / c2, w = fmaf(cy, c2, fy * c1) / c2;
        if (u >= 0.f && u < (float)v.W && w >= 0.f && w < (float)v.H) count += 1.f;
    }
    return count;
}

__global__ __launch_bounds__(256) void frustum_visibility_kernel(const NsffFrustumArgs v, const float* __restrict__ xyz,
                                                                 long long n_points, float* __restrict__ out) {
    const long long p = (long long)blockIdx.x * 256 + threadIdx.x;
    if (p < n_points) out[p] = frustum_count(v, xyz[3 * p], xyz[3 * p + 1], xyz[3 * p + 2]);
}

__global__ __launch_bounds__(64 * WAVES_PER_BLOCK) void composite_kernel(const NsffCompositeArgs a) {
    const int lane = threadIdx.x & 63;
    const long long ray = (long long)blockIdx.x * WAVES_PER_BLOCK + (threadIdx.x >> 6);
    if (ray >= a.n_rays) return;
    const int S = a.n_samples;
    const bool tr = a.has_transient != 0;
    const bool flows = tr && a.flow_mode >= 1;
    const bool warps = tr && a.flow_mode >= 2;

    float cT = 1.f, cTs = 1.f, cTfw = 1.f, cTbw = 1.f;
    float s_depth = 0.f, s_rgb[3] = {0, 0, 0}, s_talpha = 0.f, s_trgb[3] = {0, 0, 0};
    float s_sorgb[3] = {0, 0, 0}, s_sodepth = 0.f;
    float s_xyz[3] = {0, 0, 0}, s_ffw[3] = {0, 0, 0}, s_fbw[3] = {0, 0, 0};
    float s_rgbfw[3] = {0, 0, 0}, s_rgbbw[3] = {0, 0, 0}, s_occfw = 0.f, s_occbw = 0.f;

    for (int base = 0; base < S; base += 64) {
        const int i = base + lane;
        const bool on = i < S;
        const long long idx = ray * S + (on ? i : S - 1);
        const float z = a.zs[idx];
        const bool last = i >= S - 1;
        const float dz = last ? 0.f : a.zs[idx + 1] - z;
        const float d_s = last ? 100.f : dz;
        const float d_t = last ? 1e-3f : dz;
        const float* rec = a.raw + idx * RS;

        float sig_s = rec[3];
        if (a.noise_static) sig_s += a.noise_static[idx] * a.noise_std;
        sig_s = softplus(sig_s);
        const float al_s = 1.f - expf(-d_s * sig_s);
        float rgb_s[3] = {0, 0, 0};
        if (a.has_rgb) { rgb_s[0] = rec[0]; rgb_s[1] = rec[1]; rgb_s[2] = rec[2]; }

        float sig_t = 0.f, al_t = 0.f, alpha = al_s;
        float rgb_t[3] = {0, 0, 0};
        if (tr) {
            sig_t = rec[7];
            if (a.visibility && a.visibility[idx] == 0.f) sig_t = -10.f;
            if (a.vis.w2c && frustum_count(a.vis, a.xyz[idx * 3], a.xyz[idx * 3 + 1], a.xyz[idx * 3 + 2]) == 0.f) sig_t = -10.f;
            if (a.noise_transient) sig_t += a.noise_transient[idx] * a.noise_std;
            sig_t = softplus(sig_t);
            al_t = 1.f - expf(-d_t * sig_t);
            alpha = 1.f - (1.f - al_s) * (1.f - al_t);
            if (a.has_rgb) { rgb_t[0] = rec[4]; rgb_t[1] = rec[5]; rgb_t[2] = rec[6]; }
        }
        const float om = on ? 1.f - alpha : 1.f;
        const float inc = wave_scan_mul(om, lane);
        float exc = __shfl_up(inc, 1);
        if (lane == 0) exc = 1.f;
        const float T = cT * exc;
        cT *= __shfl(inc, 63);
        const float w = alpha * T, w_s = al_s * T, w_t = al_t * T;

        if (on) {
            if (a.static_sigmas) a.static_sigmas[idx] = sig_s;
            if (a.has_rgb && a.static_rgbs) {
                a.static_rgbs[idx * 3 + 0] = rgb_s[0]; a.static_rgbs[idx * 3 + 1] = rgb_s[1];
                a.static_rgbs[idx * 3 + 2] = rgb_s[2];
            }
            if (tr) {
                if (a.transient_sigmas) a.transient_sigmas[idx] = sig_t;
                if (a.has_rgb && a.transient_rgbs) {
                    a.transient_rgbs[idx * 3 + 0] = rgb_t[0]; a.transient_rgbs[idx * 3 + 1] = rgb_t[1];
                    a.transient_rgbs[idx * 3 + 2] = rgb_t[2];
                }
                if (a.static_alphas) a.static_alphas[idx] = al_s;
                if (a.transient_alphas) a.transient_alphas[idx] = al_t;
                if (a.static_weights) a.static_weights[idx] = w_s;
                if (a.transient_weights) a.transient_weights[idx] = w_t;
                if (a.weights) a.weights[idx] = w;
            } else {
                if (a.static_weights) a.static_weights[idx] = w;
                if (a.weights) a.weights[idx] = w;
            }
        }
        if (!a.has_rgb) continue;

        if (on) {
            s_depth += w * z;
            if (tr) {
#pragma unroll
                for (int c = 0; c < 3; ++c) { s_rgb[c] += w_s * rgb_s[c]; s_trgb[c] += w_t * rgb_t[c]; }
                s_talpha += w_t;
            } else {
#pragma unroll
                for (int c = 0; c < 3; ++c) s_rgb[c] += w * rgb_s[c];
            }
        }
        if (!tr) continue;

        {
            const float oms = on ? 1.f - al_s : 1.f;
            const float incs = wave_scan_mul(oms, lane);
            float excs = __shfl_up(incs, 1);
            if (lane == 0) excs = 1.f;
            const float Ts = cTs * excs;
            cTs *= __shfl(incs, 63);
            const float wso = al_s * Ts;
            if (on) {
#pragma unroll
                for (int c = 0; c < 3; ++c) s_sorgb[c] += wso * rgb_s[c];
                s_sodepth += wso * z;
            }
        }
        if (!flows) continue;

        const bool far = z > a.z_far;
        float ffw[3], fbw[3], x[3];
#pragma unroll
        for (int c = 0; c < 3; ++c) {
            ffw[c] = far ? 0.f : rec[8 + c];
            fbw[c] = far ? 0.f : rec[11 + c];
            x[c] = a.xyz[idx * 3 + c];
        }
        if (on) {
#pragma unroll
            for (int c = 0; c < 3; ++c) {
                if (a.flows_fw) a.flows_fw[idx * 3 + c] = ffw[c];
                if (a.flows_bw) a.flows_bw[idx * 3 + c] = fbw[c];
                s_xyz[c] += w * x[c]; s_ffw[c] += w * ffw[c]; s_fbw[c] += w * fbw[c];
            }
        }
        if (!warps) continue;

#pragma unroll
        for (int dir = 0; dir < 2; ++dir) {
            const float* recw = (dir == 0 ? a.raw_fw : a.raw_bw) + idx * RS;
            const float* nz = dir == 0 ? a.noise_fw : a.noise_bw;
            float sg = recw[7];
            if (nz) sg += nz[idx] * a.noise_std;
            const float al_tw = 1.f - expf(-d_t * softplus(sg));
            const float al_w = 1.f - (1.f - al_s) * (1.f - al_tw);
            const float omw = on ? 1.f - al_w : 1.f;
            const float incw = wave_scan_mul(omw, lane);
            float excw = __shfl_up(incw, 1);
            if (lane == 0) excw = 1.f;
            float& cw = dir == 0 ? cTfw : cTbw;
            const float Tw = cw * excw;
            cw *= __shfl(incw, 63);
            const float ws_w = al_s * Tw, wt_w = al_tw * Tw;
            if (on) {
                float* srgb = dir == 0 ? s_rgbfw : s_rgbbw;
#pragma unroll
                for (int c = 0; c < 3; ++c) srgb[c] += ws_w * rgb_s[c] + wt_w * recw[4 + c];
                const float* xw = (dir == 0 ? a.xyz_fw : a.xyz_bw) + idx * 3;
                float* cyc = dir == 0 ? a.xyzs_fw_bw : a.xyzs_bw_fw;
                const int head = dir == 0 ? 11 : 8;
                if (cyc) {
#pragma unroll
                    for (int c = 0; c < 3; ++c) cyc[idx * 3 + c] = xw[c] + (far ? 0.f : recw[head + c]);
                }
                const float occ = wt_w - w_t;
                if (dir == 0) { s_occfw += occ; if (a.disoccs_fw) a.disoccs_fw[idx] = 1.f - fabsf(occ); }
                else          { s_occbw += occ; if (a.disoccs_bw) a.disoccs_bw[idx] = 1.f - fabsf(occ); }
            }
        }
    }
    if (!a.has_rgb) return;

    s_depth = wave_sum(s_depth);
#pragma unroll
    for (int c = 0; c < 3; ++c) s_rgb[c] = wave_sum(s_rgb[c]);
    if (tr) {
        s_talpha = wave_sum(s_talpha); s_sodepth = wave_sum(s_sodepth);
#pragma unroll
        for (int c = 0; c < 3; ++c) { s_trgb[c] = wave_sum(s_trgb[c]); s_sorgb[c] = wave_sum(s_sorgb[c]); }
    }
    if (flows) {
#pragma unroll
        for (int c = 0; c < 3; ++c) { s_xyz[c] = wave_sum(s_xyz[c]); s_ffw[c] = wave_sum(s_ffw[c]); s_fbw[c] = wave_sum(s_fbw[c]); }
    }
    if (warps) {
        s_occfw = wave_sum(s_occfw); s_occbw = wave_sum(s_occbw);
#pragma unroll
        for (int c = 0; c < 3; ++c) { s_rgbfw[c] = wave_sum(s_rgbfw[c]); s_rgbbw[c] = wave_sum(s_rgbbw[c]); }
    }
    if (lane != 0) return;
    if (a.depth) a.depth[ray] = s_depth;
    if (!tr) {
        if (a.rgb) for (int c = 0; c < 3; ++c) a.rgb[ray * 3 + c] = s_rgb[c];
        return;
    }
    for (int c = 0; c < 3; ++c) {
        if (a.rgb) a.rgb[ray * 3 + c] = s_rgb[c] + s_trgb[c];
        if (a.transient_rgb) a.transient_rgb[ray * 3 + c] = s_trgb[c] + 0.8f * (1.f - s_talpha);
        if (a.static_only_rgb) a.static_only_rgb[ray * 3 + c] = s_sorgb[c];
    }
    if (a.transient_alpha) a.transient_alpha[ray] = s_talpha;
    if (a.static_only_depth) a.static_only_depth[ray] = s_sodepth;
    if (flows) {
        for (int c = 0; c < 3; ++c) {
            if (a.xyz_exp) a.xyz_exp[ray * 3 + c] = s_xyz[c];
            if (a.flow_fw_exp) a.flow_fw_exp[ray * 3 + c] = s_ffw[c];
            if (a.flow_bw_exp) a.flow_bw_exp[ray * 3 + c] = s_fbw[c];
            if (a.xyz_fw_exp) a.xyz_fw_exp[ray * 3 + c] = s_xyz[c] + s_ffw[c];
            if (a.xyz_bw_exp) a.xyz_bw_exp[ray * 3 + c] = s_xyz[c] + s_fbw[c];
        }
    }
    if (warps) {
        for (int c = 0; c < 3; ++c) {
            if (a.rgb_fw) a.rgb_fw[ray * 3 + c] = s_rgbfw[c];
            if (a.rgb_bw) a.rgb_bw[ray * 3 + c] = s_rgbbw[c];
        }
        if (a.disocc_fw) a.disocc_fw[ray] = 1.f - fabsf(s_occfw);
        if (a.disocc_bw) a.disocc_bw[ray] = 1.f - fabsf(s_occbw);
    }
}

template <int NCH>
__global__ __launch_bounds__(64 * NCH) void composite_kernel_chunks(const NsffCompositeArgs a) {
    __shared__ float tot[NCH][4];
    __shared__ float part[NCH][32];
    const int lane = threadIdx.x & 63, c = threadIdx.x >> 6;
    const long long ray = blockIdx.x;
    const int S = a.n_samples;
    const bool tr = a.has_transient != 0;
    const bool flows = tr && a.flow_mode >= 1;
    const bool warps = tr && a.flow_mode >= 2;

    const int i = 64 * c + lane;
    const bool on = i < S;
    const long long idx = ray * S + (on ? i : S - 1);
    const float z = a.zs[idx];
    const bool last = i >= S - 1;
    const float dz = last ? 0.f : a.zs[idx + 1] - z;
    const float d_s = last ? 100.f : dz;
    const float d_t = last ? 1e-3f : dz;
    const float* rec = a.raw + idx * RS;

    float sig_s = rec[3];
    if (a.noise_static) sig_s += a.noise_static[idx] * a.noise_std;
    sig_s = softplus(sig_s);
    const float al_s = 1.f - expf(-d_s * sig_s);
    float rgb_s[3] = {0, 0, 0};
    if (a.has_rgb) { rgb_s[0] = rec[0]; rgb_s[1] = rec[1]; rgb_s[2] = rec[2]; }

    float sig_t = 0.f, al_t = 0.f, alpha = al_s;
    float rgb_t[3] = {0, 0, 0};
    if (tr) {
        sig_t = rec[7];
        if (a.visibility && a.visibility[idx] == 0.f) sig_t = -10.f;
        if (a.vis.w2c && frustum_count(a.vis, a.xyz[idx * 3], a.xyz[idx * 3 + 1], a.xyz[idx * 3 + 2]) == 0.f) sig_t = -10.f;
        if (a.noise_transient) sig_t += a.noise_transient[idx] * a.noise_std;
        sig_t = softplus(sig_t);
        al_t = 1.f - expf(-d_t * sig_t);
        alpha = 1.f - (1.f - al_s) * (1.f - al_t);
        if (a.has_rgb) { rgb_t[0] = rec[4]; rgb_t[1] = rec[5]; rgb_t[2] = rec[6]; }
    }
    const float inc = wave_scan_mul(on ? 1.f - alpha : 1.f, lane);
    float incs = 1.f, incw[2] = {1.f, 1.f}, al_tw[2] = {0.f, 0.f};
    if (a.has_rgb && tr) incs = wave_scan_mul(on ? 1.f - al_s : 1.f, lane);
    if (a.has_rgb && warps) {
#pragma unroll
        for (int dir = 0; dir < 2; ++dir) {
            const float* recw = (dir == 0 ? a.raw_fw : a.raw_bw) + idx * RS;
            const float* nz = dir == 0 ? a.noise_fw : a.noise_bw;
            float sg = recw[7];
            if (nz) sg += nz[idx] * a.noise_std;
            al_tw[dir] = 1.f - expf(-d_t * softplus(sg));
            const float al_w = 1.f - (1.f - al_s) * (1.f - al_tw[dir]);
            incw[dir] = wave_scan_mul(on ? 1.f - al_w : 1.f, lane);
        }
    }
    if (lane == 63) { tot[c][0] = inc; tot[c][1] = incs; tot[c][2] = incw[0]; tot[c][3] = incw[1]; }
    __syncthreads();
    float cT = 1.f, cTs = 1.f, cTw[2] = {1.f, 1.f};
    for (int cc = 0; cc < c; ++cc) { cT *= tot[cc][0]; cTs *= tot[cc][1]; cTw[0] *= tot[cc][2]; cTw[1] *= tot[cc][3]; }

    float exc = __shfl_up(inc, 1);
    if (lane == 0) exc = 1.f;
    const float T = cT * exc;
    const float w = alpha * T, w_s = al_s * T, w_t = al_t * T;
    if (on) {
        if (a.static_sigmas) a.static_sigmas[idx] = sig_s;
        if (a.has_rgb && a.static_rgbs) {
            a.static_rgbs[idx * 3 + 0] = rgb_s[0]; a.static_rgbs[idx * 3 + 1] = rgb_s[1];
            a.static_rgbs[idx * 3 + 2] = rgb_s[2];
        }
        if (tr) {
            if (a.transient_sigmas) a.transient_sigmas[idx] = sig_t;
            if (a.has_rgb && a.transient_rgbs) {
                a.transient_rgbs[idx * 3 + 0] = rgb_t[0]; a.transient_rgbs[idx * 3 + 1] = rgb_t[1];
                a.transient_rgbs[idx * 3 + 2] = rgb_t[2];
            }
            if (a.static_alphas) a.static_alphas[idx] = al_s;
            if (a.transient_alphas) a.transient_alphas[idx] = al_t;
            if (a.static_weights) a.static_weights[idx] = w_s;
            if (a.transient_weights) a.transient_weights[idx] = w_t;
            if (a.weights) a.weights[idx] = w;
        } else {
            if (a.static_weights) a.static_weights[idx] = w;
            if (a.weights) a.weights[idx] = w;
        }
    }
    if (!a.has_rgb) return;

    enum { P_DEPTH, P_RGB, P_TRGB = P_RGB + 3, P_TALPHA = P_TRGB + 3, P_SORGB, P_SODEPTH = P_SORGB + 3, P_XYZ, P_FFW = P_XYZ + 3,
           P_FBW = P_FFW + 3, P_RGBFW = P_FBW + 3, P_RGBBW = P_RGBFW + 3, P_OCCFW = P_RGBBW + 3, P_OCCBW, P_N };
    static_assert(P_N <= 32, "part[] columns");
    float p[P_N];
#pragma unroll
    for (int k = 0; k < P_N; ++k) p[k] = 0.f;
    if (on) {
        p[P_DEPTH] = w * z;
        if (tr) {
#pragma unroll
            for (int k = 0; k < 3; ++k) { p[P_RGB + k] = w_s * rgb_s[k]; p[P_TRGB + k] = w_t * rgb_t[k]; }
            p[P_TALPHA] = w_t;
        } else {
#pragma unroll
            for (int k = 0; k < 3; ++k) p[P_RGB + k] = w * rgb_s[k];
        }
    }
    if (tr) {
        float excs = __shfl_up(incs, 1);
        if (lane == 0) excs = 1.f;
        const float wso = al_s * (cTs * excs);
        if (on) {
#pragma unroll
            for (int k = 0; k < 3; ++k) p[P_SORGB + k] = wso * rgb_s[k];
            p[P_SODEPTH] = wso * z;
        }
    }
    if (flows) {
        const bool far = z > a.z_far;
        float ffw[3], fbw[3], x[3];
#pragma unroll
        for (int k = 0; k < 3; ++k) {
            ffw[k] = far ? 0.f : rec[8 + k];
            fbw[k] = far ? 0.f : rec[11 + k];
            x[k] = a.xyz[idx * 3 + k];
        }
        if (on) {
#pragma unroll
            for (int k = 0; k < 3; ++k) {
                if (a.flows_fw) a.flows_fw[idx * 3 + k] = ffw[k];
                if (a.flows_bw) a.flows_bw[idx * 3 + k] = fbw[k];
                p[P_XYZ + k] = w * x[k]; p[P_FFW + k] = w * ffw[k]; p[P_FBW + k] = w * fbw[k];
            }
        }
        if (warps) {
#pragma unroll
            for (int dir = 0; dir < 2; ++dir) {
                const float* recw = (dir == 0 ? a.raw_fw : a.raw_bw) + idx * RS;
                float excw = __shfl_up(incw[dir], 1);
                if (lane == 0) excw = 1.f;
                const float Tw = cTw[dir] * excw;
                const float ws_w = al_s * Tw, wt_w = al_tw[dir] * Tw;
                if (on) {
#pragma unroll
                    for (int k = 0; k < 3; ++k) p[(dir == 0 ? P_RGBFW : P_RGBBW) + k] = ws_w * rgb_s[k] + wt_w * recw[4 + k];
                    const float* xw = (dir == 0 ? a.xyz_fw : a.xyz_bw) + idx * 3;
                    float* cyc = dir == 0 ? a.xyzs_fw_bw : a.xyzs_bw_fw;
                    const int head = dir == 0 ? 11 : 8;
                    if (cyc) {
#pragma unroll
                        for (int k = 0; k < 3; ++k) cyc[idx * 3 + k] = xw[k] + (far ? 0.f : recw[head + k]);
                    }
                    const float occ = wt_w - w_t;
                    if (dir == 0) { p[P_OCCFW] = occ; if (a.disoccs_fw) a.disoccs_fw[idx] = 1.f - fabsf(occ); }
                    else          { p[P_OCCBW] = occ; if (a.disoccs_bw) a.disoccs_bw[idx] = 1.f - fabsf(occ); }
                }
            }
        }
    }
    const int n_used = warps ? (int)P_N : (flows ? (int)P_RGBFW : (tr ? (int)P_XYZ : (int)P_TRGB));
#pragma unroll
    for (int k = 0; k < P_N; ++k) {
        if (k < n_used) {
            const float v = wave_sum(p[k]);
            if (lane == 0) part[c][k] = v;
        }
    }
    __syncthreads();
    if (threadIdx.x != 0) return;
    float s[P_N];
#pragma unroll
    for (int k = 0; k < P_N; ++k) {
        s[k] = 0.f;
        if (k < n_used) for (int cc = 0; cc < NCH; ++cc) s[k] += part[cc][k];
    }
    if (a.depth) a.depth[ray] = s[P_DEPTH];
    if (!tr) {
        if (a.rgb) for (int k = 0; k < 3; ++k) a.rgb[ray * 3 + k] = s[P_RGB + k];
        return;
    }
    for (int k = 0; k < 3; ++k) {
        if (a.rgb) a.rgb[ray * 3 + k] = s[P_RGB + k] + s[P_TRGB + k];
        if (a.transient_rgb) a.transient_rgb[ray * 3 + k] = s[P_TRGB + k] + 0.8f * (1.f - s[P_TALPHA]);
        if (a.static_only_rgb) a.static_only_rgb[ray * 3 + k] = s[P_SORGB + k];
    }
    if (a.transient_alpha) a.transient_alpha[ray] = s[P_TALPHA];
    if (a.static_only_depth) a.static_only_depth[ray] = s[P_SODEPTH];
    if (flows) {
        for (int k = 0; k < 3; ++k) {
            if (a.xyz_exp) a.xyz_exp[ray * 3 + k] = s[P_XYZ + k];
            if (a.flow_fw_exp) a.flow_fw_exp[ray * 3 + k] = s[P_FFW + k];
            if (a.flow_bw_exp) a.flow_bw_exp[ray * 3 + k] = s[P_FBW + k];
            if (a.xyz_fw_exp) a.xyz_fw_exp[ray * 3 + k] = s[P_XYZ + k] + s[P_FFW + k];
            if (a.xyz_bw_exp) a.xyz_bw_exp[ray * 3 + k] = s[P_XYZ + k] + s[P_FBW + k];
        }
    }
    if (warps) {
        for (int k = 0; k < 3; ++k) {
            if (a.rgb_fw) a.rgb_fw[ray * 3 + k] = s[P_RGBFW + k];
            if (a.rgb_bw) a.rgb_bw[ray * 3 + k] = s[P_RGBBW + k];
        }
        if (a.disocc_fw) a.disocc_fw[ray] = 1.f - fabsf(s[P_OCCFW]);
        if (a.disocc_bw) a.disocc_bw[ray] = 1.f - fabsf(s[P_OCCBW]);
    }
}

__global__ __launch_bounds__(256) void time_rows_kernel(const float* __restrict__ table, long long n_table, int width,
                                                         const long long* __restrict__ ts, long long n, long long max_t,
                                                         float* __restrict__ next, float* __restrict__ prev, int vec) {
    const int per_row = vec ? width / 4 : width;
    const long long i = (long long)blockIdx.x * 256 + threadIdx.x;
    if (i >= n * per_row) return;
    const long long r = i / per_row;
    const int c = (int)(i - r * per_row);
    const long long t = ts[r];
    long long tn = t + 1 < max_t ? t + 1 : max_t, tp = t - 1 > 0 ? t - 1 : 0;
    tn = tn < 0 ? 0 : (tn > n_table - 1 ? n_table - 1 : tn);
    tp = tp > n_table - 1 ? n_table - 1 : tp;
    if (vec) {
        if (next) reinterpret_cast<float4*>(next)[i] = reinterpret_cast<const float4*>(table + tn * width)[c];
        if (prev) reinterpret_cast<float4*>(prev)[i] = reinterpret_cast<const float4*>(table + tp * width)[c];
    } else {
        if (next) next[i] = table[tn * width + c];
        if (prev) prev[i] = table[tp * width + c];
    }
}

constexpr int TRB_CHUNK = 2048;
constexpr int TRB_COLS = 4;
__global__ __launch_bounds__(256) void time_rows_bwd_kernel(const float* __restrict__ g_cur, const float* __restrict__ g_next,
                                                             const float* __restrict__ g_prev, const long long* __restrict__ ts,
                                                             long long n, long long max_t, long long n_table, int width,
                                                             float* __restrict__ d_table) {
    __shared__ int sList[3][TRB_CHUNK];
    __shared__ int sTs[TRB_CHUNK];
    __shared__ int sCnt[3];
    __shared__ float sPart[4][64];
    const long long r = blockIdx.x;
    const int lane = threadIdx.x & 63, part = threadIdx.x >> 6;
    const float* gs[3] = {g_cur, g_next, g_prev};
    for (int cg = 0; cg < width; cg += 64 * TRB_COLS) {
        float acc[TRB_COLS];
#pragma unroll
        for (int j = 0; j < TRB_COLS; ++j) acc[j] = 0.f;
        for (long long base = 0; base < n; base += TRB_CHUNK) {
            const long long end = base + TRB_CHUNK < n ? base + TRB_CHUNK : n;
            for (long long i = base + threadIdx.x; i < end; i += 256) {
                const long long t = ts[i];
                sTs[i - base] = (int)(t < -2 ? -2 : (t > 0x7ffffff0LL ? 0x7ffffff0LL : t));
            }
            __syncthreads();
            if (part == 0) {
                int cnt[3] = {0, 0, 0};
                for (long long i0 = base; i0 < end; i0 += 64) {
                    const long long i = i0 + lane;
                    bool hit[3] = {false, false, false};
                    if (i < end) {
                        const long long t = sTs[i - base];
                        long long tn = t + 1 < max_t ? t + 1 : max_t, tp = t - 1 > 0 ? t - 1 : 0;
                        tn = tn < 0 ? 0 : (tn > n_table - 1 ? n_table - 1 : tn);
                        tp = tp > n_table - 1 ? n_table - 1 : tp;
                        hit[0] = t == r; hit[1] = tn == r; hit[2] = tp == r;
                    }
#pragma unroll
                    for (int l = 0; l < 3; ++l) {
                        const unsigned long long m = __ballot(hit[l] && gs[l] != nullptr);
                        if (hit[l] && gs[l] != nullptr) sList[l][cnt[l] + __popcll(m & ((1ull << lane) - 1ull))] = (int)(i - base);
                        cnt[l] += __popcll(m);
                    }
                }
                if (lane == 0) { sCnt[0] = cnt[0]; sCnt[1] = cnt[1]; sCnt[2] = cnt[2]; }
            }
            __syncthreads();
#pragma unroll
            for (int l = 0; l < 3; ++l) {
                const float* __restrict__ g = gs[l];
                const int cnt = sCnt[l];
                for (int k0 = part; k0 < cnt; k0 += 16) {
                    float v[4][TRB_COLS];
#pragma unroll
                    for (int u = 0; u < 4; ++u) {
                        const int k = k0 + 4 * u;
                        const float* row = g + (base + sList[l][k < cnt ? k : k0]) * width + cg + lane;
#pragma unroll
                        for (int j = 0; j < TRB_COLS; ++j)
                            v[u][j] = (k < cnt && cg + 64 * j + lane < width) ? row[64 * j] : 0.f;
                    }
#pragma unroll
                    for (int u = 0; u < 4; ++u)
#pragma unroll
                        for (int j = 0; j < TRB_COLS; ++j) acc[j] += v[u][j];
                }
            }
            __syncthreads();
        }
#pragma unroll
        for (int j = 0; j < TRB_COLS; ++j) {
            const int c = cg + 64 * j + lane;
            if (cg + 64 * j >= width) break;
            sPart[part][lane] = acc[j];
            __syncthreads();
            if (part == 0 && c < width) d_table[r * width + c] = (sPart[0][lane] + sPart[1][lane]) + (sPart[2][lane] + sPart[3][lane]);
            __syncthreads();
        }
    }
}

}

extern "C" {

int nsff_time_rows_backward(const float* g_cur, const float* g_next, const float* g_prev, const int64_t* ts, int64_t n,
                            int64_t max_t, int64_t n_table, int32_t width, float* d_table, void* stream) {
    if (n < 0 || n_table < 1 || n_table > 0x7fffffffLL || width < 1) return NSFF_ERR_INVALID;
    if (!d_table || (n > 0 && !ts)) return NSFF_ERR_NULL;
    hipLaunchKernelGGL(time_rows_bwd_kernel, dim3((unsigned)n_table), dim3(256), 0, (hipStream_t)stream, g_cur, g_next, g_prev,
                       reinterpret_cast<const long long*>(ts), (long long)n, (long long)max_t, (long long)n_table, (int)width,
                       d_table);
    return nsff_launch_status();
}

int nsff_time_rows(const float* table, int64_t n_table, int32_t width, const int64_t* ts, int64_t n, int64_t max_t,
                   float* next, float* prev, void* stream) {
    if (n < 0 || n_table < 1 || width < 1) return NSFF_ERR_INVALID;
    if (n == 0 || (!next && !prev)) return NSFF_OK;
    if (!table || !ts) return NSFF_ERR_NULL;
    const int vec = (width % 4 == 0) && !(((uintptr_t)table | (uintptr_t)next | (uintptr_t)prev) & 15);
    const long long total = n * (vec ? width / 4 : width);
    hipLaunchKernelGGL(time_rows_kernel, dim3((unsigned)((total + 255) / 256)), dim3(256), 0, (hipStream_t)stream, table,
                       (long long)n_table, (int)width, reinterpret_cast<const long long*>(ts), (long long)n, (long long)max_t,
                       next, prev, vec);
    return nsff_launch_status();
}


int nsff_coarse_samples(const float* rays, int64_t n_rays, const float* z_lin, int32_t n_samples,
                        float perturb, const float* perturb_rand, float* zs, float* xyz, void* stream) {
    if (n_rays < 0 || n_samples < 1) return NSFF_ERR_INVALID;
    if (n_rays == 0) return NSFF_OK;
    if (!rays || !z_lin || !zs || !xyz) return NSFF_ERR_NULL;
    if (perturb > 0.f && !perturb_rand) return NSFF_ERR_NULL;
    const long long total = (long long)n_rays * n_samples;
    hipLaunchKernelGGL(coarse_samples_kernel, dim3((unsigned)((total + 255) / 256)), dim3(256), 0,
                       (hipStream_t)stream, rays, (long long)n_rays, z_lin, n_samples, perturb,
                       perturb_rand, zs, xyz);
    return nsff_launch_status();
}

int nsff_fine_samples(const float* rays, int64_t n_rays, const float* z_lin, const float* zs_coarse,
                      int32_t n_samples, int32_t n_importance,
                      const float* weights_static, const float* weights_transient,
                      const float* u_static, const float* u_transient, int32_t u_per_ray,
                      float* samples_static, float* samples_transient,
                      float* zs_fine, float* xyz_fine, void* stream) {
    if (n_rays < 0 || n_samples < 3 || n_importance < 1) return NSFF_ERR_INVALID;
    if (n_rays == 0) return NSFF_OK;
    if (!rays || !z_lin || !zs_coarse || !weights_static || !u_static || !zs_fine || !xyz_fine) return NSFF_ERR_NULL;
    if (weights_transient && !u_transient) return NSFF_ERR_NULL;
    FineArgs a{rays, (long long)n_rays, z_lin, zs_coarse, n_samples, n_importance,
               weights_static, weights_transient, u_static, u_transient, u_per_ray,
               samples_static, samples_transient, zs_fine, xyz_fine};
    const int Sf = n_samples + (weights_transient ? 2 : 1) * n_importance;
    const size_t lds = (size_t)(WAVES_PER_BLOCK * n_samples + ((n_samples + 3) & ~3) + Sf) * sizeof(float);
    if (lds > 64 * 1024 || n_rays > 0x7fffffffLL) return NSFF_ERR_INVALID;
    const unsigned blocks = (unsigned)n_rays;
    hipLaunchKernelGGL(fine_samples_kernel, dim3(blocks), dim3(64 * WAVES_PER_BLOCK), lds,
                       (hipStream_t)stream, a);
    return nsff_launch_status();
}

int nsff_sample_pdf(const float* bins, const float* weights, int64_t n_rays, int32_t n_bins_minus1,
                    const float* u, int32_t n_importance, int32_t u_per_ray, float eps,
                    float* samples, void* stream) {
    if (n_rays < 0 || n_bins_minus1 < 1 || n_importance < 1) return NSFF_ERR_INVALID;
    if (n_rays == 0) return NSFF_OK;
    if (!bins || !weights || !u || !samples) return NSFF_ERR_NULL;
    PdfArgs a{bins, weights, (long long)n_rays, n_bins_minus1, u, n_importance, u_per_ray, eps, samples};
    const size_t lds = (size_t)WAVES_PER_BLOCK * (n_bins_minus1 + 1) * sizeof(float);
    if (lds > 64 * 1024) return NSFF_ERR_INVALID;
    const unsigned blocks = (unsigned)((n_rays + WAVES_PER_BLOCK - 1) / WAVES_PER_BLOCK);
    hipLaunchKernelGGL(sample_pdf_kernel, dim3(blocks), dim3(64 * WAVES_PER_BLOCK), lds,
                       (hipStream_t)stream, a);
    return nsff_launch_status();
}

int nsff_warp_points(const float* raw, const float* xyz, const float* zs, int64_t n_points,
                     float z_far, float* xyz_fw, float* xyz_bw, void* stream) {
    if (n_points < 0) return NSFF_ERR_INVALID;
    if (n_points == 0) return NSFF_OK;
    if (!raw || !xyz || !zs || !xyz_fw || !xyz_bw) return NSFF_ERR_NULL;
    const long long total = (long long)n_points * 3;
    hipLaunchKernelGGL(warp_points_kernel, dim3((unsigned)((total + 255) / 256)), dim3(256), 0,
                       (hipStream_t)stream, raw, xyz, zs, (long long)n_points, z_far, xyz_fw, xyz_bw);
    return nsff_launch_status();
}

int nsff_frame_rays(const float* K4_host, const float* c2w_host, int32_t H, int32_t W, float near, float shift_near,
                    int64_t first_pixel, int64_t n_pixels, float* rays, void* stream) {
    if (!K4_host || !c2w_host) return NSFF_ERR_NULL;
    if (H < 1 || W < 1 || first_pixel < 0 || n_pixels < 0 || first_pixel + n_pixels > (int64_t)H * W) return NSFF_ERR_INVALID;
    if (n_pixels == 0) return NSFF_OK;
    if (!rays) return NSFF_ERR_NULL;
    FrameRayArgs a{};
    a.fx = K4_host[0]; a.fy = K4_host[1]; a.cx = K4_host[2]; a.cy = K4_host[3];
    for (int i = 0; i < 12; ++i) a.c2w[i] = c2w_host[i];
    a.W = W; a.near = near; a.shift_near = shift_near; a.first = first_pixel; a.count = n_pixels; a.rays = rays;
    hipLaunchKernelGGL(frame_rays_kernel, dim3((unsigned)((n_pixels + 255) / 256)), dim3(256), 0, (hipStream_t)stream, a);
    return nsff_launch_status();
}

int nsff_composite(const NsffCompositeArgs* args, void* stream) {
    if (!args) return NSFF_ERR_NULL;
    const NsffCompositeArgs& a = *args;
    if (a.n_rays < 0 || a.n_samples < 1 || a.flow_mode < 0 || a.flow_mode > 2) return NSFF_ERR_INVALID;
    if (a.n_rays == 0) return NSFF_OK;
    if (!a.raw || !a.zs) return NSFF_ERR_NULL;
    if (a.flow_mode && (!a.has_transient || !a.has_rgb)) return NSFF_ERR_INVALID;
    if (a.flow_mode >= 1 && !a.xyz) return NSFF_ERR_NULL;
    if (a.flow_mode == 2 && (!a.raw_fw || !a.raw_bw || !a.xyz_fw || !a.xyz_bw)) return NSFF_ERR_NULL;
    if (a.vis.w2c && (!a.vis.ts || !a.xyz)) return NSFF_ERR_NULL;
    if (a.vis.w2c && (a.vis.n_cams < 1 || a.vis.n_frames < 1)) return NSFF_ERR_INVALID;
    const int nch = (a.n_samples + 63) / 64;
    if (nch >= 2 && nch <= 4 && a.n_rays <= 0x7fffffffLL && getenv("NSFF_SERIAL_COMPOSITE") == nullptr) {
        const dim3 grid((unsigned)a.n_rays);
        if (nch == 2) hipLaunchKernelGGL(composite_kernel_chunks<2>, grid, dim3(128), 0, (hipStream_t)stream, a);
        else if (nch == 3) hipLaunchKernelGGL(composite_kernel_chunks<3>, grid, dim3(192), 0, (hipStream_t)stream, a);
        else hipLaunchKernelGGL(composite_kernel_chunks<4>, grid, dim3(256), 0, (hipStream_t)stream, a);
        return nsff_launch_status();
    }
    const unsigned blocks = (unsigned)((a.n_rays + WAVES_PER_BLOCK - 1) / WAVES_PER_BLOCK);
    hipLaunchKernelGGL(composite_kernel, dim3(blocks), dim3(64 * WAVES_PER_BLOCK), 0,
                       (hipStream_t)stream, a);
    return nsff_launch_status();
}

int nsff_frustum_visibility(const NsffFrustumArgs* vis, const float* xyz, int64_t n_points, float* vis_count,
                            void* stream) {
    if (!vis || !vis->w2c || !vis->ts) return NSFF_ERR_NULL;
    if (n_points < 0 || vis->n_cams < 1 || vis->n_frames < 1) return NSFF_ERR_INVALID;
    if (n_points == 0) return NSFF_OK;
    if (!xyz || !vis_count) return NSFF_ERR_NULL;
    const long long blocks = (n_points + 255) / 256;
    if (blocks > 0x7fffffffLL) return NSFF_ERR_INVALID;
    hipLaunchKernelGGL(frustum_visibility_kernel, dim3((unsigned)blocks), dim3(256), 0, (hipStream_t)stream, *vis, xyz,
                       (long long)n_points, vis_count);
    return nsff_launch_status();
}

}
```

### nsff_pl_amd/rendering.py

```python
import os

import torch

from . import _lib
from . import autograd
from . import config
from . import range_check
from . import field_grad
from . import ray_geometry

Z_FAR = 0.95

def _new(ref, *shape):
    return torch.empty(*shape, device=ref.device, dtype=torch.float32)


def sample_pdf(bins, weights, N_importance, det=False, eps=1e-5):
    _lib.require_gpu_tensor(bins, "sample_pdf bins")
    bins = bins.contiguous().float()
    weights = weights.contiguous().float()
    n_rays = weights.shape[0]
    if det:
        u = torch.linspace(0, 1, N_importance, device=bins.device)
    else:
        u = torch.rand(n_rays, N_importance, device=bins.device)
    out = _new(bins, n_rays, N_importance)
    if n_rays:
        _lib.sample_pdf(bins, weights, u.contiguous(), 0 if det else 1, eps, out)
    return out


_TORCH_RAND, _TORCH_RANDN = torch.rand, torch.randn


class _Draws:

    def __init__(self, device, n_rays, N_samples, N_importance, perturb, noise_std, test_time, models, kwargs, coarse=None):
        self.device = device
        self.coarse_done = False
        self.fused = (device.type == "cuda" and torch.rand is _TORCH_RAND and torch.randn is _TORCH_RANDN
                      and not os.environ.get("NSFF_TORCH_RNG") and not torch.cuda.is_current_stream_capturing()
                      and _lib.fused_draws_match_torch(device))
        self.at = 0
        if not self.fused:
            return
        first = models["coarse"] if N_importance > 0 else models["fine"]
        transient = bool(kwargs.get("output_transient", True) and first.encode_transient)
        flows = kwargs.get("output_transient_flow", []) if transient else []
        noisy = float(noise_std) != 0
        plan, need = [], []

        def add(kind, need_values, *shape):
            plan.append((kind, shape))
            need.append(bool(need_values))
        hook = None
        if perturb > 0:
            add("rand", coarse is None, n_rays, N_samples)
            if coarse is not None and n_rays:
                hook = (coarse[0], coarse[1], float(perturb), coarse[2], coarse[3])
        S = N_samples
        if N_importance > 0:
            add("randn", noisy, n_rays, S)
            if transient:
                add("randn", noisy, n_rays, S)
            if perturb != 0:
                add("rand", True, n_rays, N_importance)
                if transient:
                    add("rand", True, n_rays, N_importance)
            S = N_samples + (2 if transient else 1) * N_importance
        add("randn", noisy, n_rays, S)
        if transient:
            add("randn", noisy, n_rays, S)
            if flows and not test_time:
                add("randn", noisy, n_rays, S)
                add("randn", noisy, n_rays, S)
        self.plan = plan
        self.values = _lib.fused_draws(plan, device, need, coarse=hook)
        self.coarse_done = hook is not None

    def take(self, kind, *shape):
        if not self.fused:
            return (torch.rand if kind == "rand" else torch.randn)(*shape, device=self.device)
        if self.at >= len(self.plan) or self.plan[self.at] != (kind, shape):
            raise RuntimeError(f"draw {self.at}: {kind}{shape} is not the planned {self.plan[self.at:self.at + 1]}")
        self.at += 1
        return self.values[self.at - 1]


class _Pass:
    __slots__ = ("embeddings", "rays", "ts", "max_t", "noise_std", "test_time", "kwargs",
                 "freqs_xyz", "dir_embedded", "n_rays", "rec", "tbias", "neighbour_rows", "draws")


def _embed_rows(embeddings, key, idx):
    return embeddings[key](idx).detach().contiguous().float()


_LINSPACE = {}


def _unit_linspace(n, device):
    key = (int(n), str(device))
    if key not in _LINSPACE:
        if len(_LINSPACE) > 64:
            _LINSPACE.clear()
        _LINSPACE[key] = torch.linspace(0, 1, n, device=device)
    return _LINSPACE[key]


def _neighbour_time_rows(embeddings, ts, max_t):
    m = embeddings['t']
    if (isinstance(m, torch.nn.Embedding) and m.padding_idx is None and m.max_norm is None and m.weight.is_cuda
            and m.weight.dtype == torch.float32 and m.weight.is_contiguous() and ts.is_cuda and ts.dtype == torch.int64):
        return _lib.time_rows(m.weight.detach(), ts.contiguous(), max_t)
    return (_embed_rows(embeddings, 't', torch.clamp(ts + 1, max=max_t)),
            _embed_rows(embeddings, 't', torch.clamp(ts - 1, min=0)))


def _time_codes(ctx, models, kwargs, N_samples, N_importance, output_transient, flows):
    ctx.tbias, ctx.neighbour_rows = {}, None
    if not output_transient:
        return None
    n_rays, ts, m = ctx.n_rays, ctx.ts, ctx.embeddings.get('t')
    override = kwargs.get('t_embedded') if 't_embedded' in kwargs else None
    plan = []
    if not (ctx.rec is not None or n_rays == 0 or config.get_precision() != "f16x3" or config.get_tile_points() not in (0, 130)):
        passes = [('coarse', N_samples), ('fine', N_samples + 2 * N_importance)] if N_importance > 0 else [('fine', N_samples)]
        for typ, S in passes:
            model = models[typ]
            if not model.encode_transient or S % 64 or (n_rays * S < 32768 and config.get_tile_points() == 0):
                continue
            if model.in_channels_t > 64 or model.in_channels_t % 4:
                continue
            if typ == 'fine' and flows and not ctx.test_time and hasattr(model, "transient_flow_fw"):
                plan += [(typ, 'fw', model, 1), (typ, 'bw', model, -1)]
            plan.append((typ, 't', model, 0))
    plain = (override is None and isinstance(m, torch.nn.Embedding) and m.padding_idx is None and m.max_norm is None
             and m.weight.is_cuda and m.weight.dtype == torch.float32 and m.weight.is_contiguous()
             and torch.is_tensor(ts) and ts.is_cuda and ts.dtype == torch.int64
             and ts.dim() == 1 and ts.shape[0] == n_rays)
    if (plan and plain and all(mod.in_channels_t == m.weight.shape[1] for _, _, mod, _ in plan)
            and not os.environ.get('NSFF_NO_TIME_INDEX')):
        outs, rows = _lib.time_bias([(mod, d) for _, _, mod, d in plan], index=(m.weight.detach(), ts.contiguous(), ctx.max_t))
        for (typ, which, _, _), out in zip(plan, outs):
            ctx.tbias[(typ, which)] = out
        if 1 in rows:
            ctx.neighbour_rows = (rows[1], rows[-1])
        return rows[0]
    t_embedded = override if override is not None else ctx.embeddings['t'](ts)
    t_embedded = t_embedded.detach().contiguous().float()
    plan = [p for p in plan if t_embedded.shape == (n_rays, p[2].in_channels_t)]
    if plan:
        if any(w == 'fw' for _, w, _, _ in plan):
            ctx.neighbour_rows = _neighbour_time_rows(ctx.embeddings, ts, ctx.max_t)
        src = {0: t_embedded, 1: ctx.neighbour_rows[0] if ctx.neighbour_rows else None, -1: ctx.neighbour_rows[1] if ctx.neighbour_rows else None}
        for (typ, which, _, _), out in zip(plan, _lib.time_bias([(mod, src[d]) for _, _, mod, d in plan])):
            ctx.tbias[(typ, which)] = out
    return t_embedded


def _inference(results, ctx, model, xyz, zs, output_transient, output_transient_flow,
               t_embedded, a_embedded):
    typ = model.typ
    n_rays, S = zs.shape
    test_time = ctx.test_time
    results[f'zs_{typ}'] = zs
    results[f'xyzs_{typ}'] = xyz
    P = n_rays * S
    sigma_only = typ == 'coarse' and test_time
    want_flow = bool(output_transient_flow) and output_transient and not sigma_only
    warps = want_flow and not test_time
    disocc = warps and 'disocc' in output_transient_flow
    if want_flow and not hasattr(model, "transient_flow_fw"):
        raise AttributeError(f"{typ} model has no flow heads")

    raw = _new(zs, P, _lib.RAW_STRIDE)
    side = dict(dir_emb=ctx.dir_embedded if model.use_viewdir and not sigma_only else None,
                a_emb=a_embedded if (model.use_viewdir and model.in_channels_a > 0 and not sigma_only) else None)
    big_enough = ctx.rec is not None or config.get_tile_points() == 130 or (config.get_tile_points() == 0 and P >= 32768)
    if (side["dir_emb"] is not None and P and S % 64 == 0 and config.get_precision() == "f16x3" and config.get_tile_points() in (0, 130)
            and big_enough and not os.environ.get('NSFF_NO_SIDE_BIAS')):
        side["s_bias"] = _lib.side_bias(model, side["dir_emb"], side["a_emb"])

    def query(tag, raw_out, pts, static_mode, transient_mode, flow_heads, t_rows, which='t', **extra):
        saves = {}
        if ctx.rec is not None and field_grad.forward_can_save(model, static_mode, transient_mode):
            x3 = config.grad_x3()
            acts, xin, masks, side_rows = field_grad.alloc_saves(model, P, zs.device, bool(transient_mode), bool(static_mode), x3)
            saves = dict(save_acts=acts, save_xin=xin, save_masks=masks, save_side=side_rows, save_lo=x3)
            ctx.rec.setdefault("saved", {})[tag] = (raw_out, acts, xin, masks, pts.view(-1, 3), side_rows, x3)
        t_bias = ctx.tbias.get((typ, which)) if (transient_mode and not saves) else None
        _lib.field_query(model, raw_out, P, S, static_mode=static_mode, transient_mode=transient_mode,
                         flow_heads=flow_heads, xyz=pts, freqs=ctx.freqs_xyz, t_emb=t_rows, t_bias=t_bias, **saves, **extra)
    if P:
        query(typ, raw, xyz, 1 if sigma_only else 2, 0 if not output_transient else (1 if sigma_only else 2),
              2 if want_flow else 0, t_embedded if output_transient else None, **side)

    vis = None
    if test_time and output_transient and 'dataset' in ctx.kwargs and P:
        vis = ray_geometry.frustum_args(ctx.kwargs['dataset'], ctx.ts, zs.device)

    nstd = float(ctx.noise_std)
    noise_s = ctx.draws.take("randn", n_rays, S)
    noise_t = ctx.draws.take("randn", n_rays, S) if output_transient else None
    if ctx.rec is not None and nstd != 0:
        ctx.rec[f"{typ}_static"], ctx.rec[f"{typ}_transient"] = noise_s, noise_t

    args = dict(n_rays=n_rays, n_samples=S, has_transient=int(output_transient),
                has_rgb=int(not sigma_only), flow_mode=0, want_disocc=int(disocc),
                noise_std=nstd, z_far=Z_FAR, raw=raw, zs=zs, xyz=xyz, vis=vis,
                noise_static=noise_s if nstd != 0 else None,
                noise_transient=noise_t if (nstd != 0 and output_transient) else None)

    def out(key, *shape):
        t = _new(zs, *shape)
        results[key] = t
        return t

    if not sigma_only:
        args['static_rgbs'] = out(f'static_rgbs_{typ}', n_rays, S, 3)
        if output_transient:
            args['transient_rgbs'] = out(f'transient_rgbs_{typ}', n_rays, S, 3)
            if want_flow:
                args['flows_fw'] = out('transient_flows_fw', n_rays, S, 3)
                args['flows_bw'] = out('transient_flows_bw', n_rays, S, 3)
    args['static_sigmas'] = out(f'static_sigmas_{typ}', n_rays, S)
    if output_transient:
        args['transient_sigmas'] = out(f'transient_sigmas_{typ}', n_rays, S)

    if warps:
        ts = ctx.ts
        xyz_w = _new(zs, 2, n_rays, S, 3)
        xyz_fw, xyz_bw = xyz_w[0], xyz_w[1]
        results['xyzs_fw'] = xyz_fw
        raw_w = _new(zs, 2 * P, _lib.RAW_STRIDE)
        raw_fw, raw_bw = raw_w[:P], raw_w[P:]
        tp1, tm1 = ctx.neighbour_rows if ctx.neighbour_rows is not None else _neighbour_time_rows(ctx.embeddings, ts, ctx.max_t)
        tb_fw, tb_bw = ctx.tbias.get((typ, 'fw')), ctx.tbias.get((typ, 'bw'))
        def halves(a, b):
            return (a.untyped_storage().data_ptr() == b.untyped_storage().data_ptr()
                    and a.data_ptr() + a.numel() * 4 == b.data_ptr())
        merged = (ctx.rec is None and P > 0 and not os.environ.get('NSFF_NO_MERGED_REQUERY') and halves(tp1, tm1)
                  and (tb_fw is None) == (tb_bw is None) and (tb_fw is None or halves(tb_fw, tb_bw)))
        if P:
            _lib.warp_points(raw, xyz, zs, Z_FAR, xyz_fw, xyz_bw)
            if merged:
                ctx.tbias[(typ, 'fwbw')] = None if tb_fw is None else torch.as_strided(tb_fw, (2 * n_rays,) + tuple(tb_fw.shape[1:]),
                                                                                         tb_fw.stride())
                _lib.field_query(model, raw_w, 2 * P, S, static_mode=0, transient_mode=2, flow_heads=1, xyz=xyz_w,
                                 freqs=ctx.freqs_xyz, t_emb=torch.as_strided(tp1, (2 * n_rays, tp1.shape[1]), tp1.stride()),
                                 t_bias=ctx.tbias[(typ, 'fwbw')])
            else:
                query(f"{typ}_warp_fw", raw_fw, xyz_fw, 0, 2, 1, tp1, which='fw')
        noise_fw = ctx.draws.take("randn", n_rays, S)
        out('rgb_fw', n_rays, 3)
        results['xyzs_bw'] = xyz_bw
        if P and not merged:
            query(f"{typ}_warp_bw", raw_bw, xyz_bw, 0, 2, 1, tm1, which='bw')
        noise_bw = ctx.draws.take("randn", n_rays, S)
        if ctx.rec is not None and nstd != 0:
            ctx.rec[f"{typ}_warp_fw"], ctx.rec[f"{typ}_warp_bw"] = noise_fw, noise_bw
        out('rgb_bw', n_rays, 3)
        args.update(raw_fw=raw_fw, raw_bw=raw_bw, xyz_fw=xyz_fw, xyz_bw=xyz_bw,
                    noise_fw=noise_fw if nstd != 0 else None,
                    noise_bw=noise_bw if nstd != 0 else None,
                    rgb_fw=results['rgb_fw'], rgb_bw=results['rgb_bw'],
                    xyzs_fw_bw=out('xyzs_fw_bw', n_rays, S, 3),
                    xyzs_bw_fw=out('xyzs_bw_fw', n_rays, S, 3))

    if output_transient:
        args['static_weights'] = out(f'static_weights_{typ}', n_rays, S)
        args['transient_weights'] = out(f'transient_weights_{typ}', n_rays, S)
        args['weights'] = out(f'weights_{typ}', n_rays, S)
    else:
        args['static_weights'] = out(f'static_weights_{typ}', n_rays, S)
    if test_time and output_transient:
        args['static_alphas'] = out(f'static_alphas_{typ}', n_rays, S)
        args['transient_alphas'] = out(f'transient_alphas_{typ}', n_rays, S)

    if not sigma_only:
        args['depth'] = out(f'depth_{typ}', n_rays)
        args['rgb'] = out(f'rgb_{typ}', n_rays, 3)
        if output_transient:
            args['transient_alpha'] = out(f'transient_alpha_{typ}', n_rays)
            args['transient_rgb'] = out(f'transient_rgb_{typ}', n_rays, 3)
            args['static_only_rgb'] = out(f'_static_rgb_{typ}', n_rays, 3)
            args['static_only_depth'] = out(f'_static_depth_{typ}', n_rays)
            if want_flow:
                args['flow_mode'] = 2 if warps else 1
                args['xyz_exp'] = out('xyz_fine', n_rays, 3)
                args['flow_fw_exp'] = out('transient_flow_fw', n_rays, 3)
                args['xyz_fw_exp'] = out('xyz_fw', n_rays, 3)
                args['flow_bw_exp'] = out('transient_flow_bw', n_rays, 3)
                args['xyz_bw_exp'] = out('xyz_bw', n_rays, 3)
                if disocc:
                    args['disocc_fw'] = out('disocc_fw', n_rays, 1)
                    args['disoccs_fw'] = out('disoccs_fw', n_rays, S, 1)
                    args['disocc_bw'] = out('disocc_bw', n_rays, 1)
                    args['disoccs_bw'] = out('disoccs_bw', n_rays, S, 1)
    if n_rays:
        _lib.composite(**args)


def render_rays(models,
                embeddings,
                rays,
                ts,
                max_t,
                N_samples=64,
                perturb=0,
                noise_std=0,
                N_importance=0,
                chunk=1024 * 32,
                test_time=False,
                **kwargs):
    _lib.require_gpu_tensor(rays, "rays")
    return range_check.checked(
        "render_rays", rays.device,
        lambda: _render_rays(models, embeddings, rays, ts, max_t, N_samples, perturb, noise_std, N_importance, chunk, test_time, kwargs),
        can_fallback=bool(test_time) and perturb == 0 and noise_std == 0)


def _render_rays(models, embeddings, rays, ts, max_t, N_samples, perturb, noise_std, N_importance, chunk, test_time, kwargs,
                 fine_points=None):
    _lib.require_gpu_tensor(rays, "rays")
    _lib.load()
    want_grad = (torch.is_grad_enabled() and not test_time and
                 bool(autograd.grad_parameters(models, embeddings)))
    rec = {} if want_grad else None
    with torch.cuda.device(rays.device), torch.no_grad():
        results = {}
        rays = rays.contiguous().float()
        n_rays = rays.shape[0]
        embedding_xyz, embedding_dir = embeddings['xyz'], embeddings['dir']

        ctx = _Pass()
        ctx.embeddings, ctx.rays, ctx.ts, ctx.max_t = embeddings, rays, ts, max_t
        ctx.noise_std, ctx.test_time, ctx.kwargs, ctx.n_rays = noise_std, test_time, kwargs, n_rays
        ctx.freqs_xyz = [float(f) for f in embedding_xyz.freqs]
        ctx.rec = rec
        ctx.tbias, ctx.neighbour_rows = {}, None
        ctx.dir_embedded = None
        if any(m.use_viewdir for m in models.values()):
            view_dir = kwargs.get('view_dir', rays[:, 3:6])
            ctx.dir_embedded = embedding_dir(view_dir.contiguous().float())

        z_lin = _unit_linspace(N_samples, rays.device)
        zs = _new(rays, n_rays, N_samples)
        xyz_coarse = _new(rays, n_rays, N_samples, 3)
        ctx.draws = _Draws(rays.device, n_rays, N_samples, N_importance, perturb, noise_std, test_time, models, kwargs,
                           coarse=(rays, z_lin, zs, xyz_coarse))
        perturb_rand = ctx.draws.take("rand", n_rays, N_samples) if perturb > 0 else None
        if n_rays and not ctx.draws.coarse_done:
            _lib.coarse_samples(rays, z_lin, perturb, perturb_rand, zs, xyz_coarse)

        t_embedded = None
        if N_importance > 0:
            model = models['coarse']
            output_transient = bool(kwargs.get('output_transient', True) and model.encode_transient)
            t_embedded = _time_codes(ctx, models, kwargs, N_samples, N_importance, output_transient,
                                     kwargs.get('output_transient_flow', []))
            _inference(results, ctx, model, xyz_coarse, zs, output_transient, [], t_embedded, None)

            det = perturb == 0
            if det:
                u_s = _unit_linspace(N_importance, rays.device)
                u_t = u_s
            else:
                u_s = ctx.draws.take("rand", n_rays, N_importance)
                u_t = ctx.draws.take("rand", n_rays, N_importance) if output_transient else None
            S_fine = N_samples + (2 if output_transient else 1) * N_importance
            zs_static = _new(rays, n_rays, N_importance) if test_time else None
            zs_transient = _new(rays, n_rays, N_importance) if (test_time and output_transient) else None
            zs_fine = _new(rays, n_rays, S_fine)
            xyz_fine = _new(rays, n_rays, S_fine, 3)
            if n_rays:
                _lib.fine_samples(rays, z_lin, zs, N_importance,
                                  results['static_weights_coarse'],
                                  results['transient_weights_coarse'] if output_transient else None,
                                  u_s, u_t if output_transient else None, 0 if det else 1,
                                  zs_static, zs_transient, zs_fine, xyz_fine)
            if test_time:
                results['static_zs_fine'] = zs_static
                if output_transient:
                    results['transient_zs_fine'] = zs_transient
            if fine_points is not None:
                zs_fine, xyz_fine = fine_points(rays, zs_fine, xyz_fine)
                if tuple(zs_fine.shape) != (n_rays, S_fine) or tuple(xyz_fine.shape) != (n_rays, S_fine, 3):
                    raise ValueError(f"fine_points: expected shapes {(n_rays, S_fine)} / {(n_rays, S_fine, 3)}")
            zs, xyz = zs_fine, xyz_fine
        else:
            xyz = xyz_coarse

        model = models['fine']
        a_embedded = None
        if model.encode_appearance:
            a_embedded = kwargs['a_embedded'] if 'a_embedded' in kwargs else embeddings['a'](ts)
            a_embedded = a_embedded.detach().contiguous().float()
        if N_importance == 0:
            output_transient = bool(kwargs.get('output_transient', True) and model.encode_transient)
            t_embedded = _time_codes(ctx, models, kwargs, N_samples, 0, output_transient, kwargs.get('output_transient_flow', []))
        output_transient_flow = [] if not output_transient else kwargs.get('output_transient_flow', [])
        _inference(results, ctx, model, xyz, zs, output_transient, output_transient_flow,
                   t_embedded, a_embedded)
    if rec is None:
        return results
    rec.update(N_importance=N_importance, noise_std=float(noise_std), output_transient=output_transient,
               flows=list(output_transient_flow), zs_coarse=results.get('zs_coarse', results.get('zs_fine')),
               zs_fine=results['zs_fine'], view_dir=kwargs.get('view_dir', rays[:, 3:6]), dir_embedded=ctx.dir_embedded,
               t_embedded_override=kwargs.get('t_embedded'), a_embedded_override=kwargs.get('a_embedded'))
    return autograd.attach(results, models, embeddings, rays, ts, max_t, rec)


from .interpolation import interpolate
```

Measured before the change: 68.20 million ray-samples/s.

## Fuse coarse composite with fine sampling and preload records in chunked composite

Adds a kernel that runs the coarse composite for a ray in one wave, keeps its weights in LDS, and then does the fine-sample PDF draw and sort in the same block. This removes a separate launch and the global round trip of the coarse weights. The chunked composite also gets a specialised, templated variant that preloads each raw record with vectorised float4 loads and resolves the feature flags at compile time. In exchange, the coarse composite now runs serially on a single wave per ray instead of the multi-wave chunked kernel, and the number of template instantiations grows.

```diff
diff --git a/include/nsff_render.h b/include/nsff_render.h
--- a/include/nsff_render.h
+++ b/include/nsff_render.h
@@ -325,6 +325,17 @@
 
 int nsff_composite(const NsffCompositeArgs* args, void* stream);
 
+int nsff_composite_fine_samples(const NsffCompositeArgs* args, const float* rays, const float* z_lin, int32_t n_importance,
+                                const float* u_static, const float* u_transient, int32_t u_per_ray,
+                                float* samples_static, float* samples_transient, float* zs_fine, float* xyz_fine, void* stream);
+
+#define NSFF_COMPOSITE_NONE              0
+#define NSFF_COMPOSITE_SERIAL            1
+#define NSFF_COMPOSITE_CHUNKS            2
+#define NSFF_COMPOSITE_WITH_FINE_SAMPLES 3
+#define NSFF_COMPOSITE_CHUNKS_PRELOAD    16
+int nsff_last_composite_kernel(void);
+
 int nsff_frustum_visibility(const NsffFrustumArgs* vis, const float* xyz, int64_t n_points, float* vis_count,
                             void* stream);
 
diff --git a/nsff_pl_amd/_lib.py b/nsff_pl_amd/_lib.py
--- a/nsff_pl_amd/_lib.py
+++ b/nsff_pl_amd/_lib.py
@@ -199,6 +199,9 @@
                                   C.c_float, _fp, _fp]),
     "nsff_warp_points": (C.c_int, [_fp, _fp, _fp, C.c_int64, C.c_float, _fp, _fp, _fp]),
     "nsff_composite": (C.c_int, [C.POINTER(CompositeArgs), _fp]),
+    "nsff_last_composite_kernel": (C.c_int, []),
+    "nsff_composite_fine_samples": (C.c_int, [C.POINTER(CompositeArgs), _fp, _fp, C.c_int32, _fp, _fp, C.c_int32,
+                                              _fp, _fp, _fp, _fp, _fp]),
     "nsff_frustum_visibility": (C.c_int, [C.POINTER(FrustumArgs), _fp, C.c_int64, _fp, _fp]),
     "nsff_frame_rays": (C.c_int, [C.POINTER(C.c_float), C.POINTER(C.c_float), C.c_int32, C.c_int32, C.c_float,
                                   C.c_float, C.c_int64, C.c_int64, _fp, _fp]),
@@ -647,7 +650,7 @@
            "nsff_frustum_visibility")
 
 
-def composite(vis=None, **kw):
+def _composite_args(vis, kw):
     a = CompositeArgs()
     for k, v in kw.items():
         if k in _COMPOSITE_PTRS_IN or k in _COMPOSITE_PTRS_OUT:
@@ -656,7 +659,25 @@
             setattr(a, k, v)
     if vis is not None:
         a.vis = vis
-    _check(load().nsff_composite(C.byref(a), _stream()), "nsff_composite")
+    return a
+
+
+def composite(vis=None, **kw):
+    _check(load().nsff_composite(C.byref(_composite_args(vis, kw)), _stream()), "nsff_composite")
+
+
+def last_composite_kernel():
+    code = load().nsff_last_composite_kernel()
+    return {0: None, 1: "serial", 2: "chunks", 3: "with_fine_samples"}.get(code, "chunks_preload")
+
+
+def composite_fine_samples(composite_kw, rays, z_lin, n_importance, u_static, u_transient, u_per_ray,
+                           samples_static, samples_transient, zs_fine, xyz_fine):
+    kw = dict(composite_kw)
+    a = _composite_args(kw.pop("vis", None), kw)
+    _check(load().nsff_composite_fine_samples(C.byref(a), _ptr(rays), _ptr(z_lin), int(n_importance), _ptr(u_static),
+                                              _ptr(u_transient), int(u_per_ray), _ptr(samples_static), _ptr(samples_transient),
+                                              _ptr(zs_fine), _ptr(xyz_fine), _stream()), "nsff_composite_fine_samples")
 
 
 def frame_rays(K4, c2w12, H, W, near, shift_near, first, count, rays):
diff --git a/nsff_pl_amd/csrc/rays.hip b/nsff_pl_amd/csrc/rays.hip
--- a/nsff_pl_amd/csrc/rays.hip
+++ b/nsff_pl_amd/csrc/rays.hip
@@ -98,24 +98,31 @@
     float* zs_fine; float* xyz_fine;
 };
 
-__global__ __launch_bounds__(64 * WAVES_PER_BLOCK) void fine_samples_kernel(const FineArgs a) {
-    extern __shared__ __attribute__((aligned(16))) float smem[];
+__host__ __device__ constexpr int fine_merged_offset(int S) { return WAVES_PER_BLOCK * S + ((S + 3) & ~3); }
+
+__device__ __forceinline__ void fine_stage(const FineArgs& a, long long ray, float* smem) {
+    constexpr int T = 64 * WAVES_PER_BLOCK;
+    const int tid = threadIdx.x, S = a.S;
+    float* bins = smem + WAVES_PER_BLOCK * S;
+    float* merged = smem + fine_merged_offset(S);
+    for (int j = tid; j < S - 1; j += T) bins[j] = 0.5f * (a.z_lin[j] + a.z_lin[j + 1]);
+    for (int j = tid; j < S; j += T) merged[j] = a.zs_coarse[ray * S + j];
+}
+
+__device__ __forceinline__ void fine_draw_sort(const FineArgs& a, long long ray, const float* ws, const float* wt, float* smem) {
     const int lane = threadIdx.x & 63, wave = threadIdx.x >> 6, tid = threadIdx.x;
     constexpr int T = 64 * WAVES_PER_BLOCK;
-    const long long ray = blockIdx.x;
     const int S = a.S, n_imp = a.n_imp;
-    const int k_sets = a.w_transient ? 2 : 1;
+    const int k_sets = wt ? 2 : 1;
     const int Sf = S + k_sets * n_imp;
     float* cdf = smem + wave * S;
     float* bins = smem + WAVES_PER_BLOCK * S;
-    float* merged = bins + ((S + 3) & ~3);
-    for (int j = tid; j < S - 1; j += T) bins[j] = 0.5f * (a.z_lin[j] + a.z_lin[j + 1]);
-    for (int j = tid; j < S; j += T) merged[j] = a.zs_coarse[ray * S + j];
+    float* merged = smem + fine_merged_offset(S);
     __syncthreads();
     {
         const bool mine = wave < k_sets;
         const int set = mine ? wave : 0;
-        const float* w = (set == 0 ? a.w_static : a.w_transient) + ray * S + 1;
+        const float* w = (set == 0 ? ws : wt) + 1;
         const float* ub = set == 0 ? a.u_static : a.u_transient;
         const float* u = a.u_per_ray ? ub + ray * n_imp : ub;
         float* keep = set == 0 ? a.samples_static : a.samples_transient;
@@ -145,6 +152,13 @@
         a.xyz_fine[dst * 3 + 1] = o1 + d1 * v;
         a.xyz_fine[dst * 3 + 2] = o2 + d2 * v;
     }
+}
+
+__global__ __launch_bounds__(64 * WAVES_PER_BLOCK) void fine_samples_kernel(const FineArgs a) {
+    extern __shared__ __attribute__((aligned(16))) float smem[];
+    const long long ray = blockIdx.x;
+    fine_stage(a, ray, smem);
+    fine_draw_sort(a, ray, a.w_static + ray * a.S, a.w_transient ? a.w_transient + ray * a.S : nullptr, smem);
 }
 
 struct PdfArgs {
@@ -241,10 +255,7 @@
     if (p < n_points) out[p] = frustum_count(v, xyz[3 * p], xyz[3 * p + 1], xyz[3 * p + 2]);
 }
 
-__global__ __launch_bounds__(64 * WAVES_PER_BLOCK) void composite_kernel(const NsffCompositeArgs a) {
-    const int lane = threadIdx.x & 63;
-    const long long ray = (long long)blockIdx.x * WAVES_PER_BLOCK + (threadIdx.x >> 6);
-    if (ray >= a.n_rays) return;
+__device__ __forceinline__ void composite_ray(const NsffCompositeArgs& a, long long ray, int lane, float* keep_ws, float* keep_wt) {
     const int S = a.n_samples;
     const bool tr = a.has_transient != 0;
     const bool flows = tr && a.flow_mode >= 1;
@@ -267,24 +278,53 @@
         const float d_t = last ? 1e-3f : dz;
         const float* rec = a.raw + idx * RS;
 
-        float sig_s = rec[3];
-        if (a.noise_static) sig_s += a.noise_static[idx] * a.noise_std;
+        float r[RS], rw[2][RS], x[3] = {0, 0, 0}, xw[2][3], nz_s = 0.f, nz_t = 0.f, nz_w[2] = {0.f, 0.f}, visible = 1.f;
+#pragma unroll
+        for (int k = 0; k < 8; ++k) r[k] = rec[k];
+        if (a.noise_static) nz_s = a.noise_static[idx];
+        if (tr) {
+            if (a.visibility) visible = a.visibility[idx];
+            if (a.noise_transient) nz_t = a.noise_transient[idx];
+        }
+        if (flows || (tr && a.vis.w2c)) {
+#pragma unroll
+            for (int c = 0; c < 3; ++c) x[c] = a.xyz[idx * 3 + c];
+        }
+        if (flows) {
+#pragma unroll
+            for (int k = 8; k < 14; ++k) r[k] = rec[k];
+        }
+        if (warps) {
+#pragma unroll
+            for (int dir = 0; dir < 2; ++dir) {
+                const float* recw = (dir == 0 ? a.raw_fw : a.raw_bw) + idx * RS;
+                const float* nz = dir == 0 ? a.noise_fw : a.noise_bw;
+#pragma unroll
+                for (int k = 4; k < 14; ++k) rw[dir][k] = recw[k];
+                if (nz) nz_w[dir] = nz[idx];
+#pragma unroll
+                for (int c = 0; c < 3; ++c) xw[dir][c] = ((dir == 0 ? a.xyz_fw : a.xyz_bw) + idx * 3)[c];
+            }
+        }
+
+        float sig_s = r[3];
+        if (a.noise_static) sig_s += nz_s * a.noise_std;
         sig_s = softplus(sig_s);
         const float al_s = 1.f - expf(-d_s * sig_s);
         float rgb_s[3] = {0, 0, 0};
-        if (a.has_rgb) { rgb_s[0] = rec[0]; rgb_s[1] = rec[1]; rgb_s[2] = rec[2]; }
+        if (a.has_rgb) { rgb_s[0] = r[0]; rgb_s[1] = r[1]; rgb_s[2] = r[2]; }
 
         float sig_t = 0.f, al_t = 0.f, alpha = al_s;
         float rgb_t[3] = {0, 0, 0};
         if (tr) {
-            sig_t = rec[7];
-            if (a.visibility && a.visibility[idx] == 0.f) sig_t = -10.f;
-            if (a.vis.w2c && frustum_count(a.vis, a.xyz[idx * 3], a.xyz[idx * 3 + 1], a.xyz[idx * 3 + 2]) == 0.f) sig_t = -10.f;
-            if (a.noise_transient) sig_t += a.noise_transient[idx] * a.noise_std;
+            sig_t = r[7];
+            if (a.visibility && visible == 0.f) sig_t = -10.f;
+            if (a.vis.w2c && frustum_count(a.vis, x[0], x[1], x[2]) == 0.f) sig_t = -10.f;
+            if (a.noise_transient) sig_t += nz_t * a.noise_std;
             sig_t = softplus(sig_t);
             al_t = 1.f - expf(-d_t * sig_t);
             alpha = 1.f - (1.f - al_s) * (1.f - al_t);
-            if (a.has_rgb) { rgb_t[0] = rec[4]; rgb_t[1] = rec[5]; rgb_t[2] = rec[6]; }
+            if (a.has_rgb) { rgb_t[0] = r[4]; rgb_t[1] = r[5]; rgb_t[2] = r[6]; }
         }
         const float om = on ? 1.f - alpha : 1.f;
         const float inc = wave_scan_mul(om, lane);
@@ -315,6 +355,7 @@
                 if (a.static_weights) a.static_weights[idx] = w;
                 if (a.weights) a.weights[idx] = w;
             }
+            if (keep_ws) { keep_ws[i] = tr ? w_s : w; keep_wt[i] = w_t; }
         }
         if (!a.has_rgb) continue;
 
@@ -348,12 +389,11 @@
         if (!flows) continue;
 
         const bool far = z > a.z_far;
-        float ffw[3], fbw[3], x[3];
+        float ffw[3], fbw[3];
 #pragma unroll
         for (int c = 0; c < 3; ++c) {
-            ffw[c] = far ? 0.f : rec[8 + c];
-            fbw[c] = far ? 0.f : rec[11 + c];
-            x[c] = a.xyz[idx * 3 + c];
+            ffw[c] = far ? 0.f : r[8 + c];
+            fbw[c] = far ? 0.f : r[11 + c];
         }
         if (on) {
 #pragma unroll
@@ -367,10 +407,9 @@
 
 #pragma unroll
         for (int dir = 0; dir < 2; ++dir) {
-            const float* recw = (dir == 0 ? a.raw_fw : a.raw_bw) + idx * RS;
             const float* nz = dir == 0 ? a.noise_fw : a.noise_bw;
-            float sg = recw[7];
-            if (nz) sg += nz[idx] * a.noise_std;
+            float sg = rw[dir][7];
+            if (nz) sg += nz_w[dir] * a.noise_std;
             const float al_tw = 1.f - expf(-d_t * softplus(sg));
             const float al_w = 1.f - (1.f - al_s) * (1.f - al_tw);
             const float omw = on ? 1.f - al_w : 1.f;
@@ -384,13 +423,12 @@
             if (on) {
                 float* srgb = dir == 0 ? s_rgbfw : s_rgbbw;
 #pragma unroll
-                for (int c = 0; c < 3; ++c) srgb[c] += ws_w * rgb_s[c] + wt_w * recw[4 + c];
-                const float* xw = (dir == 0 ? a.xyz_fw : a.xyz_bw) + idx * 3;
+                for (int c = 0; c < 3; ++c) srgb[c] += ws_w * rgb_s[c] + wt_w * rw[dir][4 + c];
                 float* cyc = dir == 0 ? a.xyzs_fw_bw : a.xyzs_bw_fw;
                 const int head = dir == 0 ? 11 : 8;
                 if (cyc) {
 #pragma unroll
-                    for (int c = 0; c < 3; ++c) cyc[idx * 3 + c] = xw[c] + (far ? 0.f : recw[head + c]);
+                    for (int c = 0; c < 3; ++c) cyc[idx * 3 + c] = xw[dir][c] + (far ? 0.f : rw[dir][head + c]);
                 }
                 const float occ = wt_w - w_t;
                 if (dir == 0) { s_occfw += occ; if (a.disoccs_fw) a.disoccs_fw[idx] = 1.f - fabsf(occ); }
@@ -449,16 +487,45 @@
     }
 }
 
-template <int NCH>
+__global__ __launch_bounds__(64 * WAVES_PER_BLOCK) void composite_kernel(const NsffCompositeArgs a) {
+    const long long ray = (long long)blockIdx.x * WAVES_PER_BLOCK + (threadIdx.x >> 6);
+    if (ray >= a.n_rays) return;
+    composite_ray(a, ray, threadIdx.x & 63, nullptr, nullptr);
+}
+
+__global__ __launch_bounds__(64 * WAVES_PER_BLOCK) void composite_fine_samples_kernel(const NsffCompositeArgs c, const FineArgs a) {
+    extern __shared__ __attribute__((aligned(16))) float smem[];
+    const long long ray = blockIdx.x;
+    const int S = a.S;
+    float* keep = smem + fine_merged_offset(S) + S + (c.has_transient ? 2 : 1) * a.n_imp;
+    fine_stage(a, ray, smem);
+    if ((threadIdx.x >> 6) == 0) composite_ray(c, ray, threadIdx.x & 63, keep, keep + S);
+    fine_draw_sort(a, ray, keep, c.has_transient ? keep + S : nullptr, smem);
+}
+
+enum { CH_TR = 1, CH_FLOWS = 2, CH_WARPS = 4, CH_NOISE = 8 };
+
+__device__ __forceinline__ void load_record(float (&r)[RS], const float* rec) {
+    static_assert(RS == 16, "four 16-byte loads per record");
+#pragma unroll
+    for (int q = 0; q < 4; ++q) {
+        const float4 v = reinterpret_cast<const float4*>(rec)[q];
+        r[4 * q] = v.x; r[4 * q + 1] = v.y; r[4 * q + 2] = v.z; r[4 * q + 3] = v.w;
+    }
+}
+
+template <int NCH, int SPEC>
 __global__ __launch_bounds__(64 * NCH) void composite_kernel_chunks(const NsffCompositeArgs a) {
     __shared__ float tot[NCH][4];
     __shared__ float part[NCH][32];
+    constexpr bool PRE = SPEC >= 0;
     const int lane = threadIdx.x & 63, c = threadIdx.x >> 6;
     const long long ray = blockIdx.x;
     const int S = a.n_samples;
-    const bool tr = a.has_transient != 0;
-    const bool flows = tr && a.flow_mode >= 1;
-    const bool warps = tr && a.flow_mode >= 2;
+    const bool has_rgb = PRE ? true : a.has_rgb != 0;
+    const bool tr = PRE ? (SPEC & CH_TR) != 0 : a.has_transient != 0;
+    const bool flows = PRE ? (SPEC & CH_FLOWS) != 0 : tr && a.flow_mode >= 1;
+    const bool warps = PRE ? (SPEC & CH_WARPS) != 0 : tr && a.flow_mode >= 2;
 
     const int i = 64 * c + lane;
     const bool on = i < S;
@@ -470,35 +537,60 @@
     const float d_t = last ? 1e-3f : dz;
     const float* rec = a.raw + idx * RS;
 
-    float sig_s = rec[3];
-    if (a.noise_static) sig_s += a.noise_static[idx] * a.noise_std;
+    float pr[RS], prw[2][RS], px[3], pxw[2][3], pn_s = 0.f, pn_t = 0.f, pn_w[2] = {0.f, 0.f};
+    if constexpr (PRE) {
+        load_record(pr, rec);
+        if (SPEC & CH_NOISE) { pn_s = a.noise_static[idx]; if (tr) pn_t = a.noise_transient[idx]; }
+        if (flows) {
+#pragma unroll
+            for (int k = 0; k < 3; ++k) px[k] = a.xyz[idx * 3 + k];
+        }
+        if (warps) {
+#pragma unroll
+            for (int dir = 0; dir < 2; ++dir) {
+                load_record(prw[dir], (dir == 0 ? a.raw_fw : a.raw_bw) + idx * RS);
+                if (SPEC & CH_NOISE) pn_w[dir] = (dir == 0 ? a.noise_fw : a.noise_bw)[idx];
+#pragma unroll
+                for (int k = 0; k < 3; ++k) pxw[dir][k] = ((dir == 0 ? a.xyz_fw : a.xyz_bw) + idx * 3)[k];
+            }
+        }
+    }
+    const auto R = [&](int k) { if constexpr (PRE) return pr[k]; else return rec[k]; };
+
+    float sig_s = R(3);
+    if constexpr (PRE) { if (SPEC & CH_NOISE) sig_s += pn_s * a.noise_std; }
+    else if (a.noise_static) sig_s += a.noise_static[idx] * a.noise_std;
     sig_s = softplus(sig_s);
     const float al_s = 1.f - expf(-d_s * sig_s);
     float rgb_s[3] = {0, 0, 0};
-    if (a.has_rgb) { rgb_s[0] = rec[0]; rgb_s[1] = rec[1]; rgb_s[2] = rec[2]; }
+    if (has_rgb) { rgb_s[0] = R(0); rgb_s[1] = R(1); rgb_s[2] = R(2); }
 
     float sig_t = 0.f, al_t = 0.f, alpha = al_s;
     float rgb_t[3] = {0, 0, 0};
     if (tr) {
-        sig_t = rec[7];
-        if (a.visibility && a.visibility[idx] == 0.f) sig_t = -10.f;
-        if (a.vis.w2c && frustum_count(a.vis, a.xyz[idx * 3], a.xyz[idx * 3 + 1], a.xyz[idx * 3 + 2]) == 0.f) sig_t = -10.f;
-        if (a.noise_transient) sig_t += a.noise_transient[idx] * a.noise_std;
+        sig_t = R(7);
+        if constexpr (PRE) { if (SPEC & CH_NOISE) sig_t += pn_t * a.noise_std; }
+        else {
+            if (a.visibility && a.visibility[idx] == 0.f) sig_t = -10.f;
+            if (a.vis.w2c && frustum_count(a.vis, a.xyz[idx * 3], a.xyz[idx * 3 + 1], a.xyz[idx * 3 + 2]) == 0.f) sig_t = -10.f;
+            if (a.noise_transient) sig_t += a.noise_transient[idx] * a.noise_std;
+        }
         sig_t = softplus(sig_t);
         al_t = 1.f - expf(-d_t * sig_t);
         alpha = 1.f - (1.f - al_s) * (1.f - al_t);
-        if (a.has_rgb) { rgb_t[0] = rec[4]; rgb_t[1] = rec[5]; rgb_t[2] = rec[6]; }
+        if (has_rgb) { rgb_t[0] = R(4); rgb_t[1] = R(5); rgb_t[2] = R(6); }
     }
     const float inc = wave_scan_mul(on ? 1.f - alpha : 1.f, lane);
     float incs = 1.f, incw[2] = {1.f, 1.f}, al_tw[2] = {0.f, 0.f};
-    if (a.has_rgb && tr) incs = wave_scan_mul(on ? 1.f - al_s : 1.f, lane);
-    if (a.has_rgb && warps) {
+    if (has_rgb && tr) incs = wave_scan_mul(on ? 1.f - al_s : 1.f, lane);
+    if (has_rgb && warps) {
 #pragma unroll
         for (int dir = 0; dir < 2; ++dir) {
             const float* recw = (dir == 0 ? a.raw_fw : a.raw_bw) + idx * RS;
             const float* nz = dir == 0 ? a.noise_fw : a.noise_bw;
-            float sg = recw[7];
-            if (nz) sg += nz[idx] * a.noise_std;
+            float sg;
+            if constexpr (PRE) { sg = prw[dir][7]; if (SPEC & CH_NOISE) sg += pn_w[dir] * a.noise_std; }
+            else { sg = recw[7]; if (nz) sg += nz[idx] * a.noise_std; }
             al_tw[dir] = 1.f - expf(-d_t * softplus(sg));
             const float al_w = 1.f - (1.f - al_s) * (1.f - al_tw[dir]);
             incw[dir] = wave_scan_mul(on ? 1.f - al_w : 1.f, lane);
@@ -515,13 +607,13 @@
     const float w = alpha * T, w_s = al_s * T, w_t = al_t * T;
     if (on) {
         if (a.static_sigmas) a.static_sigmas[idx] = sig_s;
-        if (a.has_rgb && a.static_rgbs) {
+        if (has_rgb && a.static_rgbs) {
             a.static_rgbs[idx * 3 + 0] = rgb_s[0]; a.static_rgbs[idx * 3 + 1] = rgb_s[1];
             a.static_rgbs[idx * 3 + 2] = rgb_s[2];
         }
         if (tr) {
             if (a.transient_sigmas) a.transient_sigmas[idx] = sig_t;
-            if (a.has_rgb && a.transient_rgbs) {
+            if (has_rgb && a.transient_rgbs) {
                 a.transient_rgbs[idx * 3 + 0] = rgb_t[0]; a.transient_rgbs[idx * 3 + 1] = rgb_t[1];
                 a.transient_rgbs[idx * 3 + 2] = rgb_t[2];
             }
@@ -535,7 +627,7 @@
             if (a.weights) a.weights[idx] = w;
         }
     }
-    if (!a.has_rgb) return;
+    if (!has_rgb) return;
 
     enum { P_DEPTH, P_RGB, P_TRGB = P_RGB + 3, P_TALPHA = P_TRGB + 3, P_SORGB, P_SODEPTH = P_SORGB + 3, P_XYZ, P_FFW = P_XYZ + 3,
            P_FBW = P_FFW + 3, P_RGBFW = P_FBW + 3, P_RGBBW = P_RGBFW + 3, P_OCCFW = P_RGBBW + 3, P_OCCBW, P_N };
@@ -569,9 +661,9 @@
         float ffw[3], fbw[3], x[3];
 #pragma unroll
         for (int k = 0; k < 3; ++k) {
-            ffw[k] = far ? 0.f : rec[8 + k];
-            fbw[k] = far ? 0.f : rec[11 + k];
-            x[k] = a.xyz[idx * 3 + k];
+            ffw[k] = far ? 0.f : R(8 + k);
+            fbw[k] = far ? 0.f : R(11 + k);
+            if constexpr (PRE) x[k] = px[k]; else x[k] = a.xyz[idx * 3 + k];
         }
         if (on) {
 #pragma unroll
@@ -585,19 +677,21 @@
 #pragma unroll
             for (int dir = 0; dir < 2; ++dir) {
                 const float* recw = (dir == 0 ? a.raw_fw : a.raw_bw) + idx * RS;
+                const float* xw = (dir == 0 ? a.xyz_fw : a.xyz_bw) + idx * 3;
+                const auto RW = [&](int k) { if constexpr (PRE) return prw[dir][k]; else return recw[k]; };
+                const auto XW = [&](int k) { if constexpr (PRE) return pxw[dir][k]; else return xw[k]; };
                 float excw = __shfl_up(incw[dir], 1);
                 if (lane == 0) excw = 1.f;
                 const float Tw = cTw[dir] * excw;
                 const float ws_w = al_s * Tw, wt_w = al_tw[dir] * Tw;
                 if (on) {
 #pragma unroll
-                    for (int k = 0; k < 3; ++k) p[(dir == 0 ? P_RGBFW : P_RGBBW) + k] = ws_w * rgb_s[k] + wt_w * recw[4 + k];
-                    const float* xw = (dir == 0 ? a.xyz_fw : a.xyz_bw) + idx * 3;
+                    for (int k = 0; k < 3; ++k) p[(dir == 0 ? P_RGBFW : P_RGBBW) + k] = ws_w * rgb_s[k] + wt_w * RW(4 + k);
                     float* cyc = dir == 0 ? a.xyzs_fw_bw : a.xyzs_bw_fw;
                     const int head = dir == 0 ? 11 : 8;
                     if (cyc) {
 #pragma unroll
-                        for (int k = 0; k < 3; ++k) cyc[idx * 3 + k] = xw[k] + (far ? 0.f : recw[head + k]);
+                        for (int k = 0; k < 3; ++k) cyc[idx * 3 + k] = XW(k) + (far ? 0.f : RW(head + k));
                     }
                     const float occ = wt_w - w_t;
                     if (dir == 0) { p[P_OCCFW] = occ; if (a.disoccs_fw) a.disoccs_fw[idx] = 1.f - fabsf(occ); }
@@ -754,9 +848,36 @@
     }
 }
 
+template <int SPEC>
+void launch_chunks(int nch, const NsffCompositeArgs& a, void* stream) {
+    const dim3 grid((unsigned)a.n_rays);
+    if (nch == 2) hipLaunchKernelGGL((composite_kernel_chunks<2, SPEC>), grid, dim3(128), 0, (hipStream_t)stream, a);
+    else if (nch == 3) hipLaunchKernelGGL((composite_kernel_chunks<3, SPEC>), grid, dim3(192), 0, (hipStream_t)stream, a);
+    else hipLaunchKernelGGL((composite_kernel_chunks<4, SPEC>), grid, dim3(256), 0, (hipStream_t)stream, a);
+}
+
+int chunks_spec(const NsffCompositeArgs& a) {
+    if (!a.has_rgb || a.visibility || a.vis.w2c) return -1;
+    const bool tr = a.has_transient != 0, warps = tr && a.flow_mode >= 2;
+    uintptr_t align = (uintptr_t)a.raw;
+    int n_draws = (a.noise_static != nullptr) + (tr && a.noise_transient != nullptr);
+    int n_wanted = tr ? 2 : 1;
+    if (warps) {
+        align |= (uintptr_t)a.raw_fw | (uintptr_t)a.raw_bw;
+        n_draws += (a.noise_fw != nullptr) + (a.noise_bw != nullptr);
+        n_wanted += 2;
+    }
+    if ((align & 15) || (n_draws != 0 && n_draws != n_wanted)) return -1;
+    return (tr ? CH_TR : 0) | (tr && a.flow_mode >= 1 ? CH_FLOWS : 0) | (warps ? CH_WARPS : 0) | (n_draws ? CH_NOISE : 0);
+}
+
+int g_last_composite = NSFF_COMPOSITE_NONE;
+
 }
 
 extern "C" {
+
+int nsff_last_composite_kernel(void) { return g_last_composite; }
 
 int nsff_time_rows_backward(const float* g_cur, const float* g_next, const float* g_prev, const int64_t* ts, int64_t n,
                             int64_t max_t, int64_t n_table, int32_t width, float* d_table, void* stream) {
@@ -809,7 +930,7 @@
                weights_static, weights_transient, u_static, u_transient, u_per_ray,
                samples_static, samples_transient, zs_fine, xyz_fine};
     const int Sf = n_samples + (weights_transient ? 2 : 1) * n_importance;
-    const size_t lds = (size_t)(WAVES_PER_BLOCK * n_samples + ((n_samples + 3) & ~3) + Sf) * sizeof(float);
+    const size_t lds = (size_t)(fine_merged_offset(n_samples) + Sf) * sizeof(float);
     if (lds > 64 * 1024 || n_rays > 0x7fffffffLL) return NSFF_ERR_INVALID;
     const unsigned blocks = (unsigned)n_rays;
     hipLaunchKernelGGL(fine_samples_kernel, dim3(blocks), dim3(64 * WAVES_PER_BLOCK), lds,
@@ -870,15 +991,52 @@
     if (a.vis.w2c && (a.vis.n_cams < 1 || a.vis.n_frames < 1)) return NSFF_ERR_INVALID;
     const int nch = (a.n_samples + 63) / 64;
     if (nch >= 2 && nch <= 4 && a.n_rays <= 0x7fffffffLL && getenv("NSFF_SERIAL_COMPOSITE") == nullptr) {
-        const dim3 grid((unsigned)a.n_rays);
-        if (nch == 2) hipLaunchKernelGGL(composite_kernel_chunks<2>, grid, dim3(128), 0, (hipStream_t)stream, a);
-        else if (nch == 3) hipLaunchKernelGGL(composite_kernel_chunks<3>, grid, dim3(192), 0, (hipStream_t)stream, a);
-        else hipLaunchKernelGGL(composite_kernel_chunks<4>, grid, dim3(256), 0, (hipStream_t)stream, a);
+        const int spec = getenv("NSFF_NO_STAGE_FUSION") == nullptr ? chunks_spec(a) : -1;
+        g_last_composite = spec < 0 ? NSFF_COMPOSITE_CHUNKS : NSFF_COMPOSITE_CHUNKS_PRELOAD + spec;
+        switch (spec) {
+            case CH_TR: launch_chunks<CH_TR>(nch, a, stream); break;
+            case CH_TR | CH_NOISE: launch_chunks<CH_TR | CH_NOISE>(nch, a, stream); break;
+            case CH_TR | CH_FLOWS: launch_chunks<CH_TR | CH_FLOWS>(nch, a, stream); break;
+            case CH_TR | CH_FLOWS | CH_NOISE: launch_chunks<CH_TR | CH_FLOWS | CH_NOISE>(nch, a, stream); break;
+            case CH_TR | CH_FLOWS | CH_WARPS: launch_chunks<CH_TR | CH_FLOWS | CH_WARPS>(nch, a, stream); break;
+            case CH_TR | CH_FLOWS | CH_WARPS | CH_NOISE: launch_chunks<CH_TR | CH_FLOWS | CH_WARPS | CH_NOISE>(nch, a, stream); break;
+            case 0: launch_chunks<0>(nch, a, stream); break;
+            case CH_NOISE: launch_chunks<CH_NOISE>(nch, a, stream); break;
+            default: launch_chunks<-1>(nch, a, stream); break;
+        }
         return nsff_launch_status();
     }
+    g_last_composite = NSFF_COMPOSITE_SERIAL;
     const unsigned blocks = (unsigned)((a.n_rays + WAVES_PER_BLOCK - 1) / WAVES_PER_BLOCK);
     hipLaunchKernelGGL(composite_kernel, dim3(blocks), dim3(64 * WAVES_PER_BLOCK), 0,
                        (hipStream_t)stream, a);
+    return nsff_launch_status();
+}
+
+int nsff_composite_fine_samples(const NsffCompositeArgs* args, const float* rays, const float* z_lin, int32_t n_importance,
+                                const float* u_static, const float* u_transient, int32_t u_per_ray,
+                                float* samples_static, float* samples_transient, float* zs_fine, float* xyz_fine, void* stream) {
+    if (!args) return NSFF_ERR_NULL;
+    const NsffCompositeArgs& c = *args;
+    if (c.n_rays < 0 || c.n_samples < 3 || c.n_samples > 64 || n_importance < 1 || c.flow_mode < 0 || c.flow_mode > 2) return NSFF_ERR_INVALID;
+    if (c.n_rays == 0) return NSFF_OK;
+    if (!c.raw || !c.zs) return NSFF_ERR_NULL;
+    if (c.flow_mode && (!c.has_transient || !c.has_rgb)) return NSFF_ERR_INVALID;
+    if (c.flow_mode >= 1 && !c.xyz) return NSFF_ERR_NULL;
+    if (c.flow_mode == 2 && (!c.raw_fw || !c.raw_bw || !c.xyz_fw || !c.xyz_bw)) return NSFF_ERR_NULL;
+    if (c.vis.w2c && (!c.vis.ts || !c.xyz)) return NSFF_ERR_NULL;
+    if (c.vis.w2c && (c.vis.n_cams < 1 || c.vis.n_frames < 1)) return NSFF_ERR_INVALID;
+    if (!rays || !z_lin || !c.static_weights || !u_static || !zs_fine || !xyz_fine) return NSFF_ERR_NULL;
+    if (c.has_transient && (!c.transient_weights || !u_transient)) return NSFF_ERR_NULL;
+    FineArgs a{rays, (long long)c.n_rays, z_lin, c.zs, c.n_samples, n_importance,
+               c.static_weights, c.has_transient ? c.transient_weights : nullptr, u_static, u_transient, u_per_ray,
+               samples_static, c.has_transient ? samples_transient : nullptr, zs_fine, xyz_fine};
+    const int Sf = c.n_samples + (c.has_transient ? 2 : 1) * n_importance;
+    const size_t lds = (size_t)(fine_merged_offset(c.n_samples) + Sf + 2 * c.n_samples) * sizeof(float);
+    if (lds > 64 * 1024 || c.n_rays > 0x7fffffffLL) return NSFF_ERR_INVALID;
+    g_last_composite = NSFF_COMPOSITE_WITH_FINE_SAMPLES;
+    hipLaunchKernelGGL(composite_fine_samples_kernel, dim3((unsigned)c.n_rays), dim3(64 * WAVES_PER_BLOCK), lds,
+                       (hipStream_t)stream, c, a);
     return nsff_launch_status();
 }
 
diff --git a/nsff_pl_amd/rendering.py b/nsff_pl_amd/rendering.py
--- a/nsff_pl_amd/rendering.py
+++ b/nsff_pl_amd/rendering.py
@@ -89,7 +89,8 @@
 
 class _Pass:
     __slots__ = ("embeddings", "rays", "ts", "max_t", "noise_std", "test_time", "kwargs",
-                 "freqs_xyz", "dir_embedded", "n_rays", "rec", "tbias", "neighbour_rows", "draws")
+                 "freqs_xyz", "dir_embedded", "n_rays", "rec", "tbias", "neighbour_rows", "draws",
+                 "hold_composite", "held_composite")
 
 
 def _embed_rows(embeddings, key, idx):
@@ -299,7 +300,10 @@
                     args['disocc_bw'] = out('disocc_bw', n_rays, 1)
                     args['disoccs_bw'] = out('disoccs_bw', n_rays, S, 1)
     if n_rays:
-        _lib.composite(**args)
+        if ctx.hold_composite:
+            ctx.held_composite = args
+        else:
+            _lib.composite(**args)
 
 
 def render_rays(models,
@@ -340,6 +344,7 @@
         ctx.freqs_xyz = [float(f) for f in embedding_xyz.freqs]
         ctx.rec = rec
         ctx.tbias, ctx.neighbour_rows = {}, None
+        ctx.hold_composite, ctx.held_composite = False, None
         ctx.dir_embedded = None
         if any(m.use_viewdir for m in models.values()):
             view_dir = kwargs.get('view_dir', rays[:, 3:6])
@@ -360,7 +365,10 @@
             output_transient = bool(kwargs.get('output_transient', True) and model.encode_transient)
             t_embedded = _time_codes(ctx, models, kwargs, N_samples, N_importance, output_transient,
                                      kwargs.get('output_transient_flow', []))
+            ctx.hold_composite = (3 <= N_samples <= 64 and fine_points is None
+                                  and not os.environ.get('NSFF_NO_STAGE_FUSION'))
             _inference(results, ctx, model, xyz_coarse, zs, output_transient, [], t_embedded, None)
+            ctx.hold_composite = False
 
             det = perturb == 0
             if det:
@@ -374,7 +382,12 @@
             zs_transient = _new(rays, n_rays, N_importance) if (test_time and output_transient) else None
             zs_fine = _new(rays, n_rays, S_fine)
             xyz_fine = _new(rays, n_rays, S_fine, 3)
-            if n_rays:
+            if n_rays and ctx.held_composite is not None:
+                _lib.composite_fine_samples(ctx.held_composite, rays, z_lin, N_importance,
+                                            u_s, u_t if output_transient else None, 0 if det else 1,
+                                            zs_static, zs_transient, zs_fine, xyz_fine)
+                ctx.held_composite = None
+            elif n_rays:
                 _lib.fine_samples(rays, z_lin, zs, N_importance,
                                   results['static_weights_coarse'],
                                   results['transient_weights_coarse'] if output_transient else None,
```

Measured after the change: 68.22 million ray-samples/s (median of 4 runs). About the same (+0.0%).
